# klausondrag/FOSVOS

Hardware: AMD Instinct MI355X
Metric: online fine-tune frames/sec (854x480) (higher is better)
Workload: dtype bf16; 1 GPU; OSVOS_VGG train_online one-shot fine-tune: 1x3x480x854 frame per step, fwd + class-balanced BCE + bwd, fused SGD step every 5 steps (BASELINE.json configs[1]); batch=1, avg_grad_every_n=5, activations=bf16 NHWC, fp32 accumulate, fp32 master weights, parallelism=single GPU

## Files before the change

### fosvos_amd/csrc/common.hpp

```cpp
#pragma once
#include <hip/hip_runtime.h>
#include <stdarg.h>
#include <algorithm>
#include <stdint.h>
#include <stdio.h>
#include <stdlib.h>
#include <string.h>

#include "../../include/fosvos_hip.h"

namespace fosvos {

extern thread_local char g_err[512];

inline int fail(int code, const char *fmt, ...) __attribute__((format(printf, 2, 3)));
inline int fail(int code, const char *fmt, ...) {
    va_list ap;
    va_start(ap, fmt);
    vsnprintf(g_err, sizeof(g_err), fmt, ap);
    va_end(ap);
    return code;
}

#define FOSVOS_HIP_CHECK(expr)                                                                         \
// ... 45 lines not shown
                     WgradReduceTable *reduce);
int wgrad_reduce_all(WgradReduceTable *reduce, int device, void *stream);
int wgrad_queue_reduce(const float *slabs, const float *bias_part, float *dw, float *db, int S, int S_bias, int64_t E_real,
                       int64_t E_pad, int Co, int Cor, int accumulate, WgradReduceTable *reduce, int device, void *stream);
struct HeadBwdArgs {
    const float *const *side;
    const int *hs, *ws;
    const float *const *filt, *const *filt1;
    const float *dsn_w, *fuse_w, *d_fused;
    const float *const *d_side_out;
    uint16_t *const *d_side;
    float *d_fuse_w, *d_fuse_b, *d_dsn_w, *d_dsn_b;
    int N, H, W, accumulate;
    void *workspace;
    size_t workspace_bytes;
    int device;
    int filt_uniform;
};
int head_bwd_check(const HeadBwdArgs &a);
int head_bwd_scale(const HeadBwdArgs &a, int s, void *stream);
int head_bwd_finish(const HeadBwdArgs &a, void *stream);

}
constexpr int kFosvosVggEvents = 25, kFosvosResnetEvents = 12;
struct fosvos_ctx {
    uint32_t magic;
    int device;
    hipEvent_t vgg_ev[kFosvosVggEvents];
    hipEvent_t resnet_ev[kFosvosResnetEvents];
    bool buckets_recorded;
};
constexpr uint32_t kFosvosCtxMagic = 0x58544346u;
namespace fosvos {
inline int ctx_check(const fosvos_ctx *ctx, const char *who) {
    FOSVOS_REQUIRE(ctx != nullptr, FOSVOS_E_ARG, "%s: null context (fosvos_ctx_create)", who);
    FOSVOS_REQUIRE(ctx->magic == kFosvosCtxMagic, FOSVOS_E_ARG, "%s: not a live fosvos_ctx", who);
    return FOSVOS_OK;
}

#ifdef FOSVOS_LAB_BUILD
inline const char *lab_env(const char *name) { return getenv(name); }
#else
inline const char *lab_env(const char *) { return nullptr; }
#endif
inline int lab_env_int(const char *name, int dflt) {
    const char *e = lab_env(name);
    return e ? atoi(e) : dflt;
}

bool conv_pp_applicable(int N, int H, int W, int in_ch, int out_ch);
int conv_pp_workgroups();
int conv_pp_forward(const uint16_t *x, const uint16_t *w_packed, const float *bias, uint16_t *y, uint16_t *y_pool, int N,
                    int H, int W, int Cin_pad, int Cout, int Co_pad, bool relu, hipStream_t st,
                    const uint8_t *mask_bits = nullptr);

inline int64_t cdiv(int64_t a, int64_t b) { return (a + b - 1) / b; }
inline int roundup(int a, int b) { return (a + b - 1) / b * b; }

typedef uint16_t bf16_t;
typedef __attribute__((ext_vector_type(8))) __bf16 bf16x8;
typedef __attribute__((ext_vector_type(4))) float f32x4;
typedef __attribute__((ext_vector_type(4))) short s16x4;
typedef unsigned int u32x4 __attribute__((__vector_size__(16)));

__device__ __forceinline__ uint16_t f2bf(float f) {
    __bf16 b = (__bf16)f;
    return __builtin_bit_cast(uint16_t, b);
}
__device__ __forceinline__ float bf2f(uint16_t v) { return __uint_as_float(((uint32_t)v) << 16); }
__device__ __forceinline__ uint4 repack8(const float (&f)[8]) {
    uint4 v;
    v.x = __builtin_amdgcn_perm(__float_as_uint(f[1]), __float_as_uint(f[0]), 0x07060302u);
    v.y = __builtin_amdgcn_perm(__float_as_uint(f[3]), __float_as_uint(f[2]), 0x07060302u);
    v.z = __builtin_amdgcn_perm(__float_as_uint(f[5]), __float_as_uint(f[4]), 0x07060302u);
    v.w = __builtin_amdgcn_perm(__float_as_uint(f[7]), __float_as_uint(f[6]), 0x07060302u);
    return v;
}
typedef float fosvos_f32x2 __attribute__((ext_vector_type(2)));
typedef __bf16 fosvos_bf16x2 __attribute__((ext_vector_type(2)));
__device__ __forceinline__ uint32_t pack2bf(float lo, float hi) {
    const fosvos_f32x2 v = {lo, hi};
    return __builtin_bit_cast(uint32_t, __builtin_convertvector(v, fosvos_bf16x2));
}
__device__ __forceinline__ float relu_f(float v) { return __int_as_float(max(__float_as_int(v), 0)); }
__device__ __forceinline__ void unpack8(const uint4 &v, float (&f)[8]) {
    f[0] = __uint_as_float(v.x << 16);
    f[1] = __uint_as_float(v.x & 0xffff0000u);
    f[2] = __uint_as_float(v.y << 16);
    f[3] = __uint_as_float(v.y & 0xffff0000u);
    f[4] = __uint_as_float(v.z << 16);
    f[5] = __uint_as_float(v.z & 0xffff0000u);
    f[6] = __uint_as_float(v.w << 16);
    f[7] = __uint_as_float(v.w & 0xffff0000u);
}
__device__ __forceinline__ uint4 pack8(const float (&f)[8]) {
    uint4 v;
    v.x = pack2bf(f[0], f[1]);
    v.y = pack2bf(f[2], f[3]);
    v.z = pack2bf(f[4], f[5]);
    v.w = pack2bf(f[6], f[7]);
    return v;
}

typedef short fosvos_i16x2 __attribute__((ext_vector_type(2)));
typedef unsigned short fosvos_u16x2 __attribute__((ext_vector_type(2)));
__device__ __forceinline__ uint32_t keep_where_pos_bf16x2(uint32_t f, uint32_t m) {
    const fosvos_i16x2 zero = {0, 0}, one = {1, 1};
// ... 91 lines not shown
```

### fosvos_amd/csrc/conv_igemm.hip

```cpp
#include <stdlib.h>

#include "common.hpp"

using namespace fosvos;

namespace {

constexpr unsigned kReluAfterAdd = 0x100u;
constexpr unsigned kSubsample2 = 0x200u;
constexpr unsigned kNoSplitK = 0x400u;

struct ConvArgs {
    const uint16_t *x;
    const uint16_t *w;
    const float *bias;
    const uint16_t *relu_src;
    const uint8_t *relu_bits;
    const uint16_t *addend;
    void *y;
    uint16_t *y_pool;
    const uint16_t *unpool_g;
    int N, H, W, Cin, Cout, Co_pad;
    int tiles_x, tiles_y;
    unsigned flags;
// ... 823 lines not shown
    if (int rc = check_common(x, w_packed, y, N, H, W, Ci, Co, "conv3x3_fwd_add")) return rc;
    FOSVOS_REQUIRE((flags & ~(FOSVOS_CONV_RELU | FOSVOS_CONV_OUT_F32)) == 0, FOSVOS_E_ARG, "conv3x3_fwd_add: unknown flags 0x%x",
                   flags);
    FOSVOS_REQUIRE(Co % 64 == 0 || Co == 32 || (Co == 16 && !addend), FOSVOS_E_SHAPE,
                   "conv3x3_fwd_add: Co=%d must be 32 or a multiple of 64 (16 without an addend)", Co);
    FOSVOS_REQUIRE(!(flags & FOSVOS_CONV_OUT_F32) || (Co == 16 && !addend), FOSVOS_E_ARG,
                   "conv3x3_fwd_add: fp32 output is the 16-channel side_prep form");
    FOSVOS_ENTER(device);
    ConvArgs a{};
    a.x = x; a.w = w_packed; a.bias = bias; a.relu_src = nullptr; a.addend = addend; a.y = y;
    a.N = N; a.H = H; a.W = W; a.Cin = roundup(Ci, 32); a.Cout = Co; a.Co_pad = roundup(Co, 16);
    a.flags = kNoSplitK | (addend ? ((flags & FOSVOS_CONV_RELU) ? kReluAfterAdd : 0u) : flags);
    return dispatch(a, Ci, workspace, workspace_bytes, (hipStream_t)stream);
}

extern "C" int fosvos_conv3x3_s2_fwd(const uint16_t *x, const uint16_t *w_packed, const float *bias, uint16_t *y, int N,
                                     int H, int W, int Ci, int Co, unsigned flags, void *workspace, size_t workspace_bytes,
                                     int device, void *stream) {
    if (int rc = check_common(x, w_packed, y, N, H, W, Ci, Co, "conv3x3_s2_fwd")) return rc;
    FOSVOS_REQUIRE((flags & ~FOSVOS_CONV_RELU) == 0, FOSVOS_E_ARG, "conv3x3_s2_fwd: unknown flags 0x%x", flags);
    FOSVOS_REQUIRE(Co % 64 == 0 || Co == 32, FOSVOS_E_SHAPE, "conv3x3_s2_fwd: Co=%d must be 32 or a multiple of 64", Co);
    FOSVOS_ENTER(device);
    ConvArgs a{};
    a.x = x; a.w = w_packed; a.bias = bias; a.relu_src = nullptr; a.addend = nullptr; a.y = y;
    a.N = N; a.H = H; a.W = W; a.Cin = roundup(Ci, 32); a.Cout = Co; a.Co_pad = roundup(Co, 16);
    a.flags = flags | kSubsample2 | kNoSplitK;
    return dispatch(a, Ci, workspace, workspace_bytes, (hipStream_t)stream);
}

extern "C" int fosvos_conv3x3_fwd_pool(const uint16_t *x, const uint16_t *w_packed, const float *bias, uint16_t *y,
                                       uint16_t *y_pool, int N, int H, int W, int Ci, int Co, unsigned flags,
                                       void *workspace, size_t workspace_bytes, int device, void *stream) {
    if (int rc = check_common(x, w_packed, y, N, H, W, Ci, Co, "conv3x3_fwd_pool")) return rc;
    FOSVOS_REQUIRE(y_pool, FOSVOS_E_ARG, "conv3x3_fwd_pool: null pooled output");
    FOSVOS_REQUIRE((flags & ~FOSVOS_CONV_RELU) == 0, FOSVOS_E_ARG, "conv3x3_fwd_pool: unknown flags 0x%x", flags);
    FOSVOS_REQUIRE(Co % 64 == 0, FOSVOS_E_SHAPE, "conv3x3_fwd_pool: Co=%d must be a multiple of 64", Co);
    if ((flags & FOSVOS_CONV_RELU) && forward_takes_pp(N, H, W, Ci, Co, flags)) {
        FOSVOS_ENTER(device);
        return conv_pp_forward(x, w_packed, bias, y, y_pool, N, H, W, roundup(Ci, 32), Co, roundup(Co, 16), true,
                               (hipStream_t)stream);
    }
    if (make_plan(N, H, W, Ci, Co).k_splits > 1) {
        if (int rc = fosvos_conv3x3_fwd(x, w_packed, bias, y, N, H, W, Ci, Co, flags, workspace, workspace_bytes, device, stream))
            return rc;
        return fosvos_maxpool2x2_ceil_fwd(y, y_pool, N, H, W, Co, device, stream);
    }
    FOSVOS_ENTER(device);
    ConvArgs a{};
    a.x = x; a.w = w_packed; a.bias = bias; a.relu_src = nullptr; a.addend = nullptr; a.y = y; a.y_pool = y_pool;
    a.N = N; a.H = H; a.W = W; a.Cin = roundup(Ci, 32); a.Cout = Co; a.Co_pad = roundup(Co, 16); a.flags = flags;
    return dispatch(a, Ci, workspace, workspace_bytes, (hipStream_t)stream);
}

extern "C" int fosvos_conv3x3_dgrad_bits(const uint16_t *dy, const uint16_t *w_dgrad_packed, const uint8_t *relu_bits,
                                         const uint16_t *addend, uint16_t *dx, int N, int H, int W, int Ci, int Co,
                                         void *workspace, size_t workspace_bytes, int device, void *stream) {
    if (int rc = check_common(dy, w_dgrad_packed, dx, N, H, W, Co, Ci, "conv3x3_dgrad_bits")) return rc;
    FOSVOS_REQUIRE(relu_bits && Ci % 8 == 0, FOSVOS_E_ARG, "conv3x3_dgrad_bits: null mask or Ci=%d not a multiple of 8", Ci);
    FOSVOS_ENTER(device);
    if (!addend && lab_env_int("FOSVOS_PP_DGRAD", 1) != 0 && lab_env_int("FOSVOS_PP", -1) != 0 &&
        conv_pp_applicable(N, H, W, roundup(Co, 32), Ci))
        return conv_pp_forward(dy, w_dgrad_packed, nullptr, dx, nullptr, N, H, W, roundup(Co, 32), Ci, roundup(Ci, 16), false,
                               (hipStream_t)stream, relu_bits);
    ConvArgs a{};
    a.x = dy; a.w = w_dgrad_packed; a.bias = nullptr; a.relu_src = nullptr; a.relu_bits = relu_bits; a.addend = addend; a.y = dx;
    a.N = N; a.H = H; a.W = W; a.Cin = roundup(Co, 32); a.Cout = Ci; a.Co_pad = roundup(Ci, 16); a.flags = 0;
    return dispatch(a, Co, workspace, workspace_bytes, (hipStream_t)stream);
}

extern "C" int fosvos_conv3x3_dgrad_unpool(const uint16_t *dy, const uint16_t *w_dgrad_packed, const uint16_t *x,
                                           const uint16_t *d_pooled, uint16_t *dx, int N, int H, int W, int Ci, int Co,
                                           void *workspace, size_t workspace_bytes, int device, void *stream) {
    if (int rc = check_common(dy, w_dgrad_packed, dx, N, H, W, Co, Ci, "conv3x3_dgrad_unpool")) return rc;
    FOSVOS_REQUIRE(x && d_pooled && x != dx, FOSVOS_E_ARG, "conv3x3_dgrad_unpool: null or aliased pooled-map operands");
    FOSVOS_ENTER(device);
    const ConvPlan plan = make_plan(N, H, W, Co, Ci);
    const bool fused = Ci % 64 == 0 && plan.k_splits == 1 && (plan.tile == kBig || plan.tile == kSquare || plan.tile == kMid) &&
                       lab_env_int("FOSVOS_UNPOOL_FUSED", 1) != 0;
    if (!fused) {
        if (int rc = fosvos_maxpool2x2_ceil_bwd(x, d_pooled, dx, N, H, W, Ci, 1, device, stream)) return rc;
        return fosvos_conv3x3_dgrad(dy, w_dgrad_packed, x, dx, dx, N, H, W, Ci, Co, workspace, workspace_bytes, device, stream);
    }
    ConvArgs a{};
    a.x = dy; a.w = w_dgrad_packed; a.relu_src = x; a.unpool_g = d_pooled; a.y = dx;
    a.N = N; a.H = H; a.W = W; a.Cin = roundup(Co, 32); a.Cout = Ci; a.Co_pad = roundup(Ci, 16); a.flags = 0;
    return dispatch(a, Co, workspace, workspace_bytes, (hipStream_t)stream);
}

extern "C" int fosvos_conv3x3_dgrad(const uint16_t *dy, const uint16_t *w_dgrad_packed, const uint16_t *relu_src,
                                    const uint16_t *addend, uint16_t *dx, int N, int H, int W, int Ci, int Co,
                                    void *workspace, size_t workspace_bytes, int device, void *stream) {
    if (int rc = check_common(dy, w_dgrad_packed, dx, N, H, W, Co, Ci, "conv3x3_dgrad")) return rc;
    FOSVOS_ENTER(device);
    ConvArgs a{};
    a.x = dy; a.w = w_dgrad_packed; a.bias = nullptr; a.relu_src = relu_src; a.addend = addend; a.y = dx;
    a.N = N; a.H = H; a.W = W; a.Cin = roundup(Co, 32); a.Cout = Ci; a.Co_pad = roundup(Ci, 16); a.flags = 0;
    return dispatch(a, Co, workspace, workspace_bytes, (hipStream_t)stream);
}
```

### fosvos_amd/csrc/conv_pp.hip

```cpp
#include <stdlib.h>

#include "common.hpp"

using namespace fosvos;

namespace fosvos {
namespace pp {

constexpr int TH = 8, TW = 32, BN = 64;
constexpr int HALO_W = TW + 2, HALO_H = TH + 2, NPIX = HALO_W * HALO_H;
constexpr int A_BYTES = NPIX * 64;
constexpr int A_PIECES = (NPIX * 4 + 63) / 64;
constexpr int W_BYTES = 36 * BN * 16;
constexpr int LDS_W = 0, LDS_A = 2 * W_BYTES, LDS_BIAS = LDS_A + 4 * A_BYTES, LDS_BYTES = LDS_BIAS + BN * 4;
constexpr int NT = 512;
static_assert(LDS_BYTES <= 160 * 1024, "one workgroup per CU");

struct Args {
    const uint16_t *x;
    const uint16_t *w;
    const float *bias;
    uint16_t *y;
    uint16_t *y_pool;
    const uint8_t *mask_bits;
    int N, H, W, Cin, Cout, Co_pad;
    int tiles_x, tiles_y, n_tiles;
    int n_cb;
    unsigned long long *stamps;
    int lab;
};
#ifdef FOSVOS_LAB_BUILD
#define PP_LAB(bit) (a.lab & (bit))
#define PP_STAMP(idx_)                                                                                            \
    if (a.stamps && blockIdx.x < 8 && wm == 0 && lane == 0 && (idx_) < 512)                                       \
        a.stamps[(blockIdx.x * 2 + g) * 512 + (idx_)] = __builtin_amdgcn_s_memtime();
#else
#define PP_LAB(bit) 0
#define PP_STAMP(idx_)
#endif

#pragma clang diagnostic push
#pragma clang diagnostic ignored "-Winline-asm"
__device__ __forceinline__ void dma16(const __amdgpu_buffer_rsrc_t rsrc, unsigned lds_dst, unsigned voff, unsigned soff) {
    asm volatile("s_mov_b32 m0, %0\n\ts_nop 4\n\tbuffer_load_dwordx4 %1, %2, %3 offen lds"
                 :: "s"(lds_dst), "v"(voff), "s"(rsrc), "s"(soff) : "memory", "m0");
}
__device__ __forceinline__ void wait_vm0() { asm volatile("s_waitcnt vmcnt(0)" ::: "memory"); }
__device__ __forceinline__ void wait_all() { asm volatile("s_waitcnt vmcnt(0) lgkmcnt(0)" ::: "memory"); }
__device__ __forceinline__ void pp_barrier() {
    asm volatile("" ::: "memory");
    __builtin_amdgcn_s_barrier();
    asm volatile("" ::: "memory");
}
#pragma clang diagnostic pop

typedef __attribute__((address_space(3))) void lds_void;
typedef __attribute__((address_space(3))) const uint4 *lds_u4_ptr;

struct TileIt {
    int idx, n, ty, tx;
    int d_n, d_ty, d_tx, stride;
    int tiles_x, tiles_y, end;
    __device__ __forceinline__ void init(int first, int stride_, int tiles_x_, int tiles_y_, int end_) {
        tiles_x = tiles_x_; tiles_y = tiles_y_; end = end_; stride = stride_;
        idx = first;
        const int per_img = tiles_x * tiles_y;
        n = first / per_img;
        const int r = first - n * per_img;
        ty = r / tiles_x;
        tx = r - ty * tiles_x;
        d_n = stride / per_img;
        const int rs = stride - d_n * per_img;
        d_ty = rs / tiles_x;
        d_tx = rs - d_ty * tiles_x;
    }
    __device__ __forceinline__ void next() {
        idx += stride;
        tx += d_tx;
        const int cx = tx >= tiles_x;
        tx -= cx ? tiles_x : 0;
        ty += d_ty + cx;
        const int cy = ty >= tiles_y;
        ty -= cy ? tiles_y : 0;
        n += d_n + cy;
    }
    __device__ __forceinline__ bool valid() const { return idx < end; }
    __device__ __forceinline__ int y0() const { return ty * TH; }
    __device__ __forceinline__ int x0() const { return tx * TW; }
};

template <bool RELU, bool POOL, bool MASK = false>
__global__ __launch_bounds__(NT) __attribute__((amdgpu_waves_per_eu(2, 2))) void k_conv3x3_pp(const Args a) {
    extern __shared__ __attribute__((aligned(16))) char smem_pp[];
    const unsigned lds0 = __builtin_amdgcn_readfirstlane((unsigned)(size_t)(lds_void *)smem_pp);
    const int tid = threadIdx.x, lane = tid & 63;
    const int wave = __builtin_amdgcn_readfirstlane(tid >> 6);
    const int g = wave >> 2, wm = wave & 3;
    const int cl = lane & 15, kq = lane >> 4;
    const int H = a.H, W = a.W, Cin = a.Cin, Cout = a.Cout;
    const int NC = Cin >> 5;

    const int b = blockIdx.x, n_wg8 = gridDim.x >> 3;
    const int xcd = b & 7, j8 = b >> 3;
    const int cb = j8 % a.n_cb, jj = j8 / a.n_cb, S = n_wg8 / a.n_cb;
    const int t_begin = (int)(((int64_t)xcd * a.n_tiles) >> 3), t_end = (int)(((int64_t)(xcd + 1) * a.n_tiles) >> 3);
    const int span = t_end - t_begin;
    const int n_it = span > 2 * jj ? (span - 2 * jj + 2 * S - 1) / (2 * S) : 0;
    if (n_it == 0) return;
    const int K = n_it * NC;
    const int n0 = cb * BN;
    TileIt cur, ldt;
    cur.init(t_begin + 2 * jj + g, 2 * S, a.tiles_x, a.tiles_y, t_end);
    ldt = cur;

    const int pj = lane >> 4, pm = lane & 15;
    const unsigned w_voff = (unsigned)(32 * (pj >> 1) + 8 * (pm >> 2) + 4 * (pj & 1) + (pm & 3)) * 16u;
    const int w_row_bytes = a.Co_pad * 16;
    const auto w_rsrc = __builtin_amdgcn_make_buffer_rsrc(const_cast<uint16_t *>(a.w), 0, NC * 36 * w_row_bytes, 0x00020000);
    auto issue_w = [&](int chunk, int buf, int first, int stride) {
        if (PP_LAB(8)) return;
        for (int r = first; r < 36; r += stride)
            dma16(w_rsrc, lds0 + LDS_W + buf * W_BYTES + r * 1024, w_voff, (unsigned)((chunk * 36 + r) * w_row_bytes + n0 * 16));
    };

    constexpr int A_IT = (A_PIECES + 3) / 4;
    int a_rel[A_IT];
#pragma unroll
    for (int i = 0; i < A_IT; ++i) {
        const int pc = wm + 4 * i;
        const int P = pc * 16 + (lane >> 2), s4 = lane & 3;
        const int hy = P / HALO_W, hx = P - hy * HALO_W;
        const int kq_src = s4 ^ ((P >> 1) & 2);
        a_rel[i] = (hy * W + hx) * Cin * 2 + kq_src * 16;
    }
    int ld_k = 0, ld_c = 0;
    int ld_base = 0, ld_edge = 0;
    __amdgpu_buffer_rsrc_t ld_rsrc;
    auto ld_open_tile = [&]() {
        if (!ldt.valid()) return;
        const int y0 = ldt.y0(), x0 = ldt.x0();
        ld_rsrc = __builtin_amdgcn_make_buffer_rsrc(const_cast<uint16_t *>(a.x) + (int64_t)ldt.n * H * W * Cin, 0,
                                                    H * W * Cin * 2, 0x00020000);
        ld_base = ((y0 - 1) * W + (x0 - 1)) * Cin * 2;
        ld_edge = !(y0 > 0 && x0 > 0 && y0 + TH < H && x0 + TW < W);
// ... 53 lines not shown
    af[i_] = __builtin_bit_cast(bf16x8, *(lds_u4_ptr)(size_t)(lds0 + LDS_A + (g * 2 + ((k_) & 1)) * A_BYTES +  \
                                                              a_sw[((i_) >> 1) + (tap_) / 3][(tap_) % 3] + ((i_) & 1) * 1024));
#define PP_RW(k_, tap_, s_, j_) \
    wf[s_][j_] = __builtin_bit_cast(bf16x8, *(lds_u4_ptr)(size_t)(w_frag0 + ((k_) & 1) * W_BYTES + (tap_) * 4096 + (j_) * 256));
#define PP_RBIAS()                                                                                            \
    _Pragma("unroll") for (int i = 0; i < 4; ++i) _Pragma("unroll") for (int j = 0; j < 4; ++j) acc[i][j] =    \
        *(__attribute__((address_space(3))) const f32x4 *)(size_t)(bias_at + (j >> 1) * 128 + (j & 1) * 16);

    uint4 pk[4][2];
    unsigned mb[MASK ? 4 : 1][2];
    int dn_n = 0, dn_y0 = 0, dn_x0 = 0;
    int st_pending = 0;
    auto pack_frag = [&](int i, int jp) {
        unsigned u[4];
#pragma unroll
        for (int e2 = 0; e2 < 4; ++e2) {
            const int e = 2 * e2;
            u[e2] = pack2bf(acc[i][2 * jp + (e >> 2)][e & 3], acc[i][2 * jp + (e >> 2)][(e & 3) + 1]);
            if constexpr (RELU) {
                const fosvos_i16x2 zero = {0, 0};
                u[e2] = __builtin_bit_cast(unsigned, __builtin_elementwise_max(__builtin_bit_cast(fosvos_i16x2, u[e2]), zero));
            }
        }
        return make_uint4(u[0], u[1], u[2], u[3]);
    };
    auto pack_tile = [&]() {
        if (!cur.valid() || PP_LAB(2)) return;
        dn_n = cur.n; dn_y0 = cur.y0(); dn_x0 = cur.x0();
        st_pending = 1;
#pragma unroll
        for (int i = 0; i < 4; ++i) {
            pk[i][0] = pack_frag(i, 0);
            pk[i][1] = pack_frag(i, 1);
        }
        if constexpr (MASK) {
            const auto m_rsrc = __builtin_amdgcn_make_buffer_rsrc(const_cast<uint8_t *>(a.mask_bits) + (int64_t)dn_n * H * W * (Cout >> 3),
                                                                  0, H * W * (Cout >> 3), 0x00020000);
#pragma unroll
            for (int i = 0; i < 4; ++i) {
                const int gy = dn_y0 + 2 * wm + (i >> 1), gx = dn_x0 + (i & 1) * 16 + cl;
                const unsigned off = (gy < H && gx < W) ? (unsigned)((gy * W + gx) * (Cout >> 3) + (n0 >> 3) + kq) : 0x80000000u;
                mb[i][0] = __builtin_amdgcn_raw_buffer_load_b8(m_rsrc, off, 0, 0);
                mb[i][1] = __builtin_amdgcn_raw_buffer_load_b8(m_rsrc, off + 4, 0, 0);
            }
        }
    };
    auto mask_bits_of = [](unsigned b) {
        return make_uint4((b & 1u) | ((b & 2u) << 15), ((b >> 2) & 1u) | ((b & 8u) << 13), ((b >> 4) & 1u) | ((b & 32u) << 11),
                          ((b >> 6) & 1u) | ((b & 128u) << 9));
    };
    auto store_slot = [&](int slot) {
        if (!st_pending) return;
        if (slot < 4) {
            const auto y_rsrc = __builtin_amdgcn_make_buffer_rsrc(a.y + (int64_t)dn_n * H * W * Cout, 0, H * W * Cout * 2, 0x00020000);
            const int gy = dn_y0 + 2 * wm + (slot >> 1), gx = dn_x0 + (slot & 1) * 16 + cl;
            const unsigned off = (gy < H && gx < W) ? (unsigned)(((gy * W + gx) * Cout + n0 + kq * 8) * 2) : 0x80000000u;
            uint4 v0 = pk[slot][0], v1 = pk[slot][1];
            if constexpr (MASK) {
                v0 = keep_where_pos_bf16x8(v0, mask_bits_of(mb[slot][0]));
                v1 = keep_where_pos_bf16x8(v1, mask_bits_of(mb[slot][1]));
            }
            __builtin_amdgcn_raw_buffer_store_b128(__builtin_bit_cast(u32x4, v0), y_rsrc, off, 0, 0);
            __builtin_amdgcn_raw_buffer_store_b128(__builtin_bit_cast(u32x4, v1), y_rsrc, off + 64, 0, 0);
        } else if constexpr (POOL) {
            const int ih = slot - 4;
            const int OH = (H + 1) >> 1, OW = (W + 1) >> 1;
            const bool edge = dn_y0 + TH > H || dn_x0 + TW > W;
            const auto p_rsrc = __builtin_amdgcn_make_buffer_rsrc(a.y_pool + (int64_t)dn_n * OH * OW * Cout, 0,
                                                                  OH * OW * Cout * 2, 0x00020000);
            const int oy = (dn_y0 >> 1) + wm, ox = (dn_x0 >> 1) + ih * 8 + (cl >> 1);
            const bool ok = !(cl & 1) && oy < OH && ox < OW;
            const unsigned off = ok ? (unsigned)(((oy * OW + ox) * Cout + n0 + kq * 8) * 2) : 0x80000000u;
#pragma unroll
            for (int jp = 0; jp < 2; ++jp) {
                uint4 top = pk[ih][jp], bot = pk[ih + 2][jp];
                if (edge) {
                    const int gy = dn_y0 + 2 * wm, gx = dn_x0 + ih * 16 + cl;
                    if (!(gy < H && gx < W)) top = make_uint4(0, 0, 0, 0);
                    if (!(gy + 1 < H && gx < W)) bot = make_uint4(0, 0, 0, 0);
                }
                const uint4 m = max_nonneg_bf16x8(top, bot);
                uint4 o;
                o.x = (unsigned)__builtin_amdgcn_update_dpp(0, (int)m.x, 0xB1, 0xF, 0xF, true);
                o.y = (unsigned)__builtin_amdgcn_update_dpp(0, (int)m.y, 0xB1, 0xF, 0xF, true);
                o.z = (unsigned)__builtin_amdgcn_update_dpp(0, (int)m.z, 0xB1, 0xF, 0xF, true);
                o.w = (unsigned)__builtin_amdgcn_update_dpp(0, (int)m.w, 0xB1, 0xF, 0xF, true);
                __builtin_amdgcn_raw_buffer_store_b128(__builtin_bit_cast(u32x4, max_nonneg_bf16x8(m, o)), p_rsrc, off + jp * 64, 0, 0);
            }
        }
    };
    constexpr int N_SLOTS = POOL ? 6 : 4;

    auto request_next = [&](int k) {
        if (k + 1 < K && (NC > 2 || k + 1 < 2)) issue_w((k + 1) % NC, (k + 1) & 1, wave, 8);
        ld_issue();
    };

    issue_w(0, 0, wave, 8);
    ld_open_tile();
    ld_issue();
    wait_all();
    pp_barrier();

#define PP_MM(tap_, i_, j_) \
    acc[i_][j_] = __builtin_amdgcn_mfma_f32_16x16x32_bf16(wf[(tap_) & 1][j_], af[i_], acc[i_][j_], 0, 0, 0);
#define PP_ROW_READS(n_, i_)                                                                                  \
    PP_RA(k, n_, i_)                                                                                          \
    if constexpr ((i_) < 2) {                                                                                 \
        PP_RW(k, n_, (n_) & 1, 2 * (i_))                                                                      \
        PP_RW(k, n_, (n_) & 1, 2 * (i_) + 1)                                                                  \
    }                                                                                                         \
    __builtin_amdgcn_sched_group_barrier(0x008, 4, 0);                                                        \
    __builtin_amdgcn_sched_group_barrier(0x002, 1, 0);                                                        \
    __builtin_amdgcn_sched_group_barrier(0x100, (i_) < 2 ? 3 : 1, 0);
#define PP_ROW(tap_, i_)                                                                                      \
    PP_MM(tap_, i_, 0) PP_MM(tap_, i_, 1) PP_MM(tap_, i_, 2) PP_MM(tap_, i_, 3)                               \
    PP_ROW_READS((tap_) + 1, i_)
#define PP_TAP(tap_) { PP_ROW(tap_, 0) PP_ROW(tap_, 1) PP_ROW(tap_, 2) PP_ROW(tap_, 3) }
#define PP_TAP_LAST()                                                                                         \
    {                                                                                                         \
// ... 26 lines not shown
            PP_BETWEEN(0) PP_BETWEEN(1) PP_BETWEEN(2) PP_BETWEEN(3) PP_BETWEEN(4) PP_BETWEEN(5) PP_BETWEEN(6) PP_BETWEEN(7) PP_BETWEEN(8)
        }
        st_pending = 0;
        if (++cp_c == NC) {
            cp_c = 0;
            pack_tile();
            cur.next();
        }
        PP_STAMP(4 * k + 2)
        wait_vm0();
        PP_STAMP(4 * k + 3)
        pp_barrier();
    }
    PP_STAMP(4 * K)
#pragma unroll
    for (int slot = 0; slot < N_SLOTS; ++slot) store_slot(slot);
#undef PP_MM
#undef PP_ROW_READS
#undef PP_ROW
#undef PP_TAP
#undef PP_TAP_LAST
#undef PP_BETWEEN
#undef PP_RA
#undef PP_RW
#undef PP_RBIAS
}

}
}

namespace fosvos {
int conv_pp_workgroups() { return 256; }
#ifdef FOSVOS_LAB_BUILD
static unsigned long long *g_pp_stamps = nullptr;
extern "C" void fosvos_lab_set_pp_stamps(void *p) { g_pp_stamps = (unsigned long long *)p; }
#endif

bool conv_pp_applicable(int N, int H, int W, int in_ch, int out_ch) {
    if (out_ch % 64 != 0 || in_ch % 32 != 0) return false;
    const int n_cb = out_ch / 64;
    if (n_cb != 1 && n_cb != 2 && n_cb != 4 && n_cb != 8) return false;
    const int64_t tiles = cdiv(W, pp::TW) * cdiv(H, pp::TH) * N;
    if (tiles > 0x3fffffff) return false;
    const int64_t units = tiles * n_cb, slots = 2 * conv_pp_workgroups();
    if (units < slots) return false;
    static const int mode = lab_env_int("FOSVOS_PP", -1);
    if (mode == 1 || in_ch <= 64) return true;
    return units * 10 >= cdiv(units, slots) * slots * 9;
}



int conv_pp_forward(const uint16_t *x, const uint16_t *w_packed, const float *bias, uint16_t *y, uint16_t *y_pool, int N,
                    int H, int W, int Cin_pad, int Cout, int Co_pad, bool relu, hipStream_t st, const uint8_t *mask_bits) {
    FOSVOS_REQUIRE(!y_pool || relu, FOSVOS_E_ARG, "conv3x3 (persistent): the fused pool takes post-ReLU values");
    FOSVOS_REQUIRE(!mask_bits || (!relu && !y_pool && !bias), FOSVOS_E_ARG, "conv3x3 (persistent): the bit mask is the data gradient's epilogue");
    pp::Args a{};
    a.x = x; a.w = w_packed; a.bias = bias; a.y = y; a.y_pool = y_pool; a.mask_bits = mask_bits;
    a.N = N; a.H = H; a.W = W; a.Cin = Cin_pad; a.Cout = Cout; a.Co_pad = Co_pad;
    a.tiles_x = (int)cdiv(W, pp::TW);
    a.tiles_y = (int)cdiv(H, pp::TH);
    a.n_tiles = a.tiles_x * a.tiles_y * N;
    a.n_cb = Cout / 64;
    a.lab = lab_env_int("FOSVOS_PP_LAB", 0);
#ifdef FOSVOS_LAB_BUILD
    a.stamps = g_pp_stamps;
#endif
    void (*kern)(const pp::Args) = mask_bits ? pp::k_conv3x3_pp<false, false, true>
                                   : y_pool  ? pp::k_conv3x3_pp<true, true>
                                   : relu    ? pp::k_conv3x3_pp<true, false> : pp::k_conv3x3_pp<false, false>;
    const int which = mask_bits ? 3 : y_pool ? 2 : relu ? 1 : 0;
    static bool once[64][4];
    int dev = 0;
    FOSVOS_HIP_CHECK(hipGetDevice(&dev));
    if (dev >= 0 && dev < 64 && !once[dev][which]) {
        FOSVOS_HIP_CHECK(hipFuncSetAttribute(reinterpret_cast<const void *>(kern), hipFuncAttributeMaxDynamicSharedMemorySize,
                                             pp::LDS_BYTES));
        once[dev][which] = true;
    }
    FOSVOS_PROF(mask_bits ? "k_conv3x3_pp<false, false, true>" : y_pool ? "k_conv3x3_pp<true, true, false>"
                : relu    ? "k_conv3x3_pp<true, false, false>" : "k_conv3x3_pp<false, false, false>", st,
                2.0 * N * H * W * 9.0 * Cin_pad * Cout);
    hipLaunchKernelGGL(kern, dim3(conv_pp_workgroups()), dim3(pp::NT), pp::LDS_BYTES, st, a);
    FOSVOS_LAUNCH_CHECK();
    return FOSVOS_OK;
}

}
```

### fosvos_amd/csrc/pool.hip

```cpp
#include "common.hpp"

using namespace fosvos;

namespace {
__global__ __launch_bounds__(256) void k_pool_fwd(const uint16_t *__restrict__ x, uint16_t *__restrict__ y, int H,
                                                   int W, int C, int OH, int OW, int64_t total) {
    const int groups = C >> 3;
    for (int64_t i = blockIdx.x * (int64_t)blockDim.x + threadIdx.x; i < total; i += (int64_t)gridDim.x * blockDim.x) {
        const int g = (int)(i % groups);
        int64_t r = i / groups;
        const int ox = (int)(r % OW);
        r /= OW;
        const int oy = (int)(r % OH);
        const int64_t n = r / OH;
        const int iy = oy * 2, ix = ox * 2;
        float m[8];
#pragma unroll
        for (int j = 0; j < 8; ++j) m[j] = -INFINITY;
#pragma unroll
        for (int dy = 0; dy < 2; ++dy)
#pragma unroll
            for (int dx = 0; dx < 2; ++dx) {
                if (iy + dy < H && ix + dx < W) {
                    const uint4 v = *reinterpret_cast<const uint4 *>(
// ... 6 lines not shown
            }
        *reinterpret_cast<uint4 *>(y + (((n * OH + oy) * OW + ox) * C + g * 8)) = pack8(m);
    }
}

__global__ __launch_bounds__(256) void k_pool_bwd(const uint16_t *__restrict__ x, const uint16_t *__restrict__ dy,
                                                   uint16_t *__restrict__ dx, int H, int W, int C, int OH, int OW,
                                                   int relu_mask) {
    const int groups = C >> 3;
    const int col = blockIdx.x * 256 + threadIdx.x;
    if (col >= OW * groups) return;
    const int ox = col / groups, g = col - ox * groups;
    const int oy = blockIdx.y;
    const int64_t n = blockIdx.z;
    const uint16_t *xn = x + n * H * W * C;
    uint16_t *dxn = dx + n * H * W * C;
    const int iy = oy * 2, ix = ox * 2;
    const bool vx = ix + 1 < W, vy = iy + 1 < H;
    const int o00 = (iy * W + ix) * C + g * 8;
    const int o01 = o00 + C, o10 = o00 + W * C, o11 = o10 + C;
    const uint4 v0 = *reinterpret_cast<const uint4 *>(xn + o00);
    const uint4 v1 = *reinterpret_cast<const uint4 *>(xn + (vx ? o01 : o00));
    const uint4 v2 = *reinterpret_cast<const uint4 *>(xn + (vy ? o10 : o00));
    const uint4 v3 = *reinterpret_cast<const uint4 *>(xn + (vx && vy ? o11 : o00));
    const uint4 gv = *reinterpret_cast<const uint4 *>(dy + ((n * OH + oy) * OW + ox) * C + g * 8);
    float x0[8], x1[8], x2[8], x3[8], gy[8];
    unpack8(v0, x0);
    unpack8(v1, x1);
    unpack8(v2, x2);
    unpack8(v3, x3);
    unpack8(gv, gy);
    float r0[8], r1[8], r2[8], r3[8];
#pragma unroll
    for (int j = 0; j < 8; ++j) {
        const float a1 = vx ? x1[j] : -INFINITY, a2 = vy ? x2[j] : -INFINITY, a3 = (vx && vy) ? x3[j] : -INFINITY;
        const bool w1 = a1 > x0[j];
        const float m1 = w1 ? a1 : x0[j];
        const bool w2 = a2 > m1;
        const float m2 = w2 ? a2 : m1;
        const bool w3 = a3 > m2;
        const float m = w3 ? a3 : m2;
        const float gval = (relu_mask && !(m > 0.f)) ? 0.f : gy[j];
        r0[j] = (w1 || w2 || w3) ? 0.f : gval;
        r1[j] = (w1 && !w2 && !w3) ? gval : 0.f;
        r2[j] = (w2 && !w3) ? gval : 0.f;
        r3[j] = w3 ? gval : 0.f;
    }
    *reinterpret_cast<uint4 *>(dxn + o00) = repack8(r0);
    if (vx) *reinterpret_cast<uint4 *>(dxn + o01) = repack8(r1);
    if (vy) *reinterpret_cast<uint4 *>(dxn + o10) = repack8(r2);
    if (vx && vy) *reinterpret_cast<uint4 *>(dxn + o11) = repack8(r3);
}

inline int grid_for(int64_t total) {
    int64_t g = cdiv(total, 256);
    if (g > 16384) g = 16384;
    if (g < 1) g = 1;
    return (int)g;
}
}

extern "C" int fosvos_maxpool2x2_ceil_fwd(const uint16_t *x, uint16_t *y, int N, int H, int W, int C, int device,
                                          void *stream) {
    FOSVOS_REQUIRE(x && y, FOSVOS_E_ARG, "maxpool_fwd: null pointer");
    FOSVOS_REQUIRE(N > 0 && H > 0 && W > 0 && C > 0 && C % 8 == 0, FOSVOS_E_SHAPE,
                   "maxpool_fwd: bad shape N=%d H=%d W=%d C=%d (C %% 8 must be 0)", N, H, W, C);
    FOSVOS_ENTER(device);
    const int OH = (H + 1) / 2, OW = (W + 1) / 2;
    const int64_t total = (int64_t)N * OH * OW * (C / 8);
    FOSVOS_PROF("k_pool_fwd", stream, 0.0);
    hipLaunchKernelGGL(k_pool_fwd, dim3(grid_for(total)), dim3(256), 0, (hipStream_t)stream, x, y, H, W, C, OH, OW, total);
    FOSVOS_LAUNCH_CHECK();
    return FOSVOS_OK;
}

extern "C" int fosvos_maxpool2x2_ceil_bwd(const uint16_t *x, const uint16_t *dy, uint16_t *dx, int N, int H, int W,
                                          int C, int relu_mask, int device, void *stream) {
    FOSVOS_REQUIRE(x && dy && dx, FOSVOS_E_ARG, "maxpool_bwd: null pointer");
    FOSVOS_REQUIRE(N > 0 && H > 0 && W > 0 && C > 0 && C % 8 == 0, FOSVOS_E_SHAPE,
                   "maxpool_bwd: bad shape N=%d H=%d W=%d C=%d (C %% 8 must be 0)", N, H, W, C);
    FOSVOS_ENTER(device);
    const int OH = (H + 1) / 2, OW = (W + 1) / 2;
    FOSVOS_REQUIRE((int64_t)H * W * C < 0x7fffffffLL && OH <= 65535 && N <= 65535, FOSVOS_E_SHAPE,
                   "maxpool_bwd: image too large (N=%d H=%d W=%d C=%d)", N, H, W, C);
    FOSVOS_PROF("k_pool_bwd", stream, 0.0);
    hipLaunchKernelGGL(k_pool_bwd, dim3((unsigned)cdiv((int64_t)OW * (C / 8), 256), (unsigned)OH, (unsigned)N), dim3(256), 0,
                       (hipStream_t)stream, x, dy, dx, H, W, C, OH, OW, relu_mask);
    FOSVOS_LAUNCH_CHECK();
    return FOSVOS_OK;
}
```

### fosvos_amd/csrc/vgg_net.hip

```cpp
#include <stdlib.h>

#include "common.hpp"

using namespace fosvos;

namespace {
constexpr int kNConv = 13;
constexpr int kStageOf[kNConv] = {0, 0, 1, 1, 2, 2, 2, 3, 3, 3, 4, 4, 4};
constexpr int kCin[kNConv] = {3, 64, 64, 128, 128, 256, 256, 256, 512, 512, 512, 512, 512};
constexpr int kCout[kNConv] = {64, 64, 128, 128, 256, 256, 256, 512, 512, 512, 512, 512, 512};
constexpr int kFirstOfStage[5] = {0, 2, 4, 7, 10};
constexpr int kLastOfStage[5] = {1, 3, 6, 9, 12};
constexpr int kStageCh[5] = {64, 128, 256, 512, 512};

inline size_t up256(size_t v) { return (v + 255) / 256 * 256; }

struct Arena {
    int sh[5], sw[5];
    size_t act[kNConv];
    size_t gact[kNConv];
    size_t pooled[4];
    size_t gpooled[4];
    size_t side[4];
    size_t dside[4];
// ... 18 lines not shown
    }
    for (int s = 1; s < 5; ++s) {
        const size_t bytes = (size_t)N * a.sh[s] * a.sw[s] * kStageCh[s - 1] * 2;
        a.pooled[s - 1] = take(bytes);
        a.gpooled[s - 1] = take(bytes);
        a.side[s - 1] = take((size_t)N * a.sh[s] * a.sw[s] * 16 * 4);
        a.dside[s - 1] = take((size_t)N * a.sh[s] * a.sw[s] * 32 * 2);
    }
    a.bits0 = take((size_t)N * H * W * (kCout[0] / 8));
    a.hws_bytes = up256(fosvos_head_bwd_workspace_bytes(N, H, W));
    a.hws = take(a.hws_bytes);
    size_t ws = 256;
    a.wsa_conv_bytes[0] = up256(fosvos_conv3x3_first_wgrad_workspace_bytes(N, H, W, 64));
    for (int c = 1; c < kNConv; ++c) {
        const int s = kStageOf[c];
        a.wsa_conv_bytes[c] = fosvos_conv3x3_wgrad_workspace_bytes(N, a.sh[s], a.sw[s], kCin[c], kCout[c]);
        if (N >= 2)
            a.wsa_conv_bytes[c] = std::max(a.wsa_conv_bytes[c],
                                           fosvos_conv3x3_workspace_bytes(N - (N + 1) / 2, a.sh[s], a.sw[s], kCin[c], kCout[c]));
        a.wsa_conv_bytes[c] = up256(a.wsa_conv_bytes[c]);
        ws = std::max(ws, fosvos_conv3x3_workspace_bytes(N, a.sh[s], a.sw[s], kCin[c], kCout[c]));
        if (N >= 2)
            ws = std::max(ws, fosvos_conv3x3_workspace_bytes((N + 1) / 2, a.sh[s], a.sw[s], kCin[c], kCout[c]));
        ws = std::max(ws, fosvos_conv3x3_workspace_bytes(N, a.sh[s], a.sw[s], kCout[c], kCin[c]));
    }
    for (int s = 1; s < 5; ++s) {
        a.wsa_side_bytes[s - 1] = up256(std::max({fosvos_conv3x3_wgrad_workspace_bytes(N, a.sh[s], a.sw[s], kStageCh[s], 16),
                                                  fosvos_conv3x3_workspace_bytes(N, a.sh[s], a.sw[s], kStageCh[s], 16),
                                                  N >= 2 ? fosvos_conv3x3_workspace_bytes(N - (N + 1) / 2, a.sh[s], a.sw[s], kStageCh[s], 16) : (size_t)0}));
        ws = std::max(ws, fosvos_conv3x3_workspace_bytes(N, a.sh[s], a.sw[s], kStageCh[s], 16));
        if (N >= 2) ws = std::max(ws, fosvos_conv3x3_workspace_bytes((N + 1) / 2, a.sh[s], a.sw[s], kStageCh[s], 16));
        ws = std::max(ws, fosvos_conv3x3_workspace_bytes(N, a.sh[s], a.sw[s], 16, kStageCh[s]));
    }
    a.ws_bytes = up256(ws);
    a.ws = take(a.ws_bytes);
    for (int c = 0; c < kNConv; ++c) a.wsa_conv[c] = take(a.wsa_conv_bytes[c]);
    for (int i = 0; i < 4; ++i) a.wsa_side[i] = take(a.wsa_side_bytes[i]);
    a.total = off;
    return a;
}

static_assert(kFosvosVggEvents == 25, "event slots below");
constexpr int kBucketFinalEvent = 22;
constexpr int kStage2WgradEvent = 23;
constexpr int kMainTailEvent = 24;
constexpr int kBucketEvent0 = 19;

#define FOSVOS_TRY(expr)          \
    do {                          \
        const int rc_ = (expr);   \
        if (rc_ != FOSVOS_OK) return rc_; \
    } while (0)

int check_net(const void *w, const void *frame, const void *arena, int N, int H, int W, size_t arena_bytes,
              const Arena &a, const char *who) {
    FOSVOS_REQUIRE(w && frame && arena, FOSVOS_E_ARG, "%s: null pointer", who);
    FOSVOS_REQUIRE(N > 0 && H > 0 && W > 0, FOSVOS_E_SHAPE, "%s: bad shape N=%d H=%d W=%d", who, N, H, W);
    FOSVOS_REQUIRE(arena_bytes >= a.total, FOSVOS_E_WORKSPACE, "%s: arena %zu < %zu bytes", who, arena_bytes, a.total);
    FOSVOS_REQUIRE(((uintptr_t)arena & 255) == 0, FOSVOS_E_ARG, "%s: arena must be 256-byte aligned", who);
    return FOSVOS_OK;
}
}

extern "C" size_t fosvos_vgg_arena_bytes(int N, int H, int W) {
    if (N <= 0 || H <= 0 || W <= 0) return 0;
    return make_arena(N, H, W).total;
}

extern "C" int fosvos_vgg_arena_layout(int N, int H, int W, fosvos_vgg_arena_layout_info *out) {
    FOSVOS_REQUIRE(out, FOSVOS_E_ARG, "vgg_arena_layout: null output");
    FOSVOS_REQUIRE(N > 0 && H > 0 && W > 0, FOSVOS_E_SHAPE, "vgg_arena_layout: bad shape N=%d H=%d W=%d", N, H, W);
    const Arena a = make_arena(N, H, W);
    *out = fosvos_vgg_arena_layout_info{};
    out->total = a.total;
    for (int s = 0; s < 5; ++s) { out->stage_h[s] = a.sh[s]; out->stage_w[s] = a.sw[s]; }
    for (int c = 0; c < kNConv; ++c) {
        const int s = kStageOf[c];
        out->act[c] = a.act[c];
        out->gact[c] = a.gact[c];
        out->act_bytes[c] = (size_t)N * a.sh[s] * a.sw[s] * kCout[c] * 2;
        out->wsa_conv[c] = a.wsa_conv[c];
        out->wsa_conv_bytes[c] = a.wsa_conv_bytes[c];
    }
    for (int s = 1; s < 5; ++s) {
        const size_t px = (size_t)N * a.sh[s] * a.sw[s];
        out->pooled[s - 1] = a.pooled[s - 1];
        out->gpooled[s - 1] = a.gpooled[s - 1];
        out->pooled_bytes[s - 1] = px * kStageCh[s - 1] * 2;
        out->side[s - 1] = a.side[s - 1];
        out->side_bytes[s - 1] = px * 16 * 4;
        out->dside[s - 1] = a.dside[s - 1];
        out->dside_bytes[s - 1] = px * 32 * 2;
        out->wsa_side[s - 1] = a.wsa_side[s - 1];
        out->wsa_side_bytes[s - 1] = a.wsa_side_bytes[s - 1];
    }
    out->bits0 = a.bits0;
    out->bits0_bytes = (size_t)N * H * W * (kCout[0] / 8);
    out->ws = a.ws; out->ws_bytes = a.ws_bytes;
    out->hws = a.hws; out->hws_bytes = a.hws_bytes;
    return FOSVOS_OK;
}

namespace {
int forward_impl(hipEvent_t *ev, const fosvos_vgg_weights *w, const float *frame, int N, int H, int W, void *arena,
                 size_t arena_bytes, float *fused, float *const side_out[4], int device, void *stream, void *aux_stream) {
    const Arena a = make_arena(N, H, W);
    FOSVOS_TRY(check_net(w, frame, arena, N, H, W, arena_bytes, a, "vgg_forward"));
    FOSVOS_REQUIRE(fused, FOSVOS_E_ARG, "vgg_forward: null output");
    char *base = reinterpret_cast<char *>(arena);
    auto act = [&](int c) { return reinterpret_cast<uint16_t *>(base + a.act[c]); };
    void *ws = base + a.ws;
    hipStream_t sm = (hipStream_t)stream;
    const bool par = ev != nullptr && aux_stream != nullptr && aux_stream != stream;
    hipStream_t sa = par ? (hipStream_t)aux_stream : sm;
    if (par) FOSVOS_ENTER(device);
    static const bool split_on = lab_env_int("FOSVOS_FWD_SPLIT", 1) != 0;
    if (split_on && N >= 2) {
        const int na = (N + 1) / 2;
        if (par) {
            FOSVOS_HIP_CHECK(hipEventRecord(ev[14], sm));
            FOSVOS_HIP_CHECK(hipStreamWaitEvent(sa, ev[14], 0));
        }
        for (int half = 0; half < 2; ++half) {
            const int f0 = half ? na : 0, nf = half ? N - na : na;
            hipStream_t st = half ? sa : sm;
            const uint16_t *xh = nullptr;
            for (int c = 0; c < kNConv; ++c) {
                const int s = kStageOf[c];
                const size_t px = (size_t)a.sh[s] * a.sw[s];
                uint16_t *yc = act(c) + (size_t)f0 * px * kCout[c];
                void *wsc = half ? base + a.wsa_conv[c] : ws;
                const size_t wsn = half ? a.wsa_conv_bytes[c] : a.ws_bytes;
                if (c == 0) {
                    FOSVOS_TRY(fosvos_conv3x3_first_fwd(frame + (size_t)f0 * 3 * H * W, w->conv_w[0], w->conv_b[0], yc,
                                                        reinterpret_cast<uint8_t *>(base + a.bits0) + (size_t)f0 * px * (kCout[0] / 8),
                                                        nf, H, W, kCout[0], device, st));
                } else {
                    if (c == kFirstOfStage[s]) {
                        const size_t ppx = (size_t)a.sh[s] * a.sw[s];
                        xh = reinterpret_cast<uint16_t *>(base + a.pooled[s - 1]) + (size_t)f0 * ppx * kCin[c];
                    }
                    FOSVOS_REQUIRE(wsn >= fosvos_conv3x3_workspace_bytes(nf, a.sh[s], a.sw[s], kCin[c], kCout[c]),
                                   FOSVOS_E_WORKSPACE, "vgg_forward: split-K workspace of the second chain");
                    if (c == kLastOfStage[s] && s < 4) {
                        const size_t qpx = (size_t)a.sh[s + 1] * a.sw[s + 1];
                        FOSVOS_TRY(fosvos_conv3x3_fwd_pool(xh, w->conv_wf[c], w->conv_b[c], yc,
                                                           reinterpret_cast<uint16_t *>(base + a.pooled[s]) + (size_t)f0 * qpx * kCout[c],
                                                           nf, a.sh[s], a.sw[s], kCin[c], kCout[c], FOSVOS_CONV_RELU, wsc, wsn,
                                                           device, st));
                    } else {
                        FOSVOS_TRY(fosvos_conv3x3_fwd(xh, w->conv_wf[c], w->conv_b[c], yc, nf, a.sh[s], a.sw[s], kCin[c],
                                                      kCout[c], FOSVOS_CONV_RELU, wsc, wsn, device, st));
                    }
                }
                xh = yc;
                if (s > 0 && c == kLastOfStage[s]) {
                    float *so = reinterpret_cast<float *>(base + a.side[s - 1]) + (size_t)f0 * px * 16;
                    FOSVOS_TRY(fosvos_conv3x3_fwd(xh, w->side_wf[s - 1], w->side_b[s - 1], so, nf, a.sh[s], a.sw[s], kStageCh[s],
                                                  16, FOSVOS_CONV_OUT_F32, half ? base + a.wsa_side[s - 1] : ws,
                                                  half ? a.wsa_side_bytes[s - 1] : a.ws_bytes, device, st));
                }
            }
        }
        static const bool head_per_chain = lab_env_int("FOSVOS_HEAD_PER_CHAIN", 1) != 0;
        if (head_per_chain) {
            for (int half = 0; half < 2; ++half) {
                const int f0 = half ? na : 0, nf = half ? N - na : na;
                const float *sideh[4];
                float *soh[4] = {nullptr, nullptr, nullptr, nullptr};
                int hsh[4], wsh[4];
                for (int i = 0; i < 4; ++i) {
                    hsh[i] = a.sh[i + 1];
                    wsh[i] = a.sw[i + 1];
                    sideh[i] = reinterpret_cast<const float *>(base + a.side[i]) + (size_t)f0 * hsh[i] * wsh[i] * 16;
                    if (side_out && side_out[i]) soh[i] = side_out[i] + (size_t)f0 * H * W;
                }
                FOSVOS_TRY(fosvos_head_fwd(sideh, hsh, wsh, w->filt, w->filt1, w->dsn_w, w->dsn_b, w->fuse_w, w->fuse_b,
                                           fused + (size_t)f0 * H * W, (side_out && side_out[0]) ? soh : nullptr, nf, H, W,
                                           w->filt_uniform, device, half ? sa : sm));
            }
        }
        if (par) {
            FOSVOS_HIP_CHECK(hipEventRecord(ev[13], sa));
            FOSVOS_HIP_CHECK(hipStreamWaitEvent(sm, ev[13], 0));
        }
        if (head_per_chain) return FOSVOS_OK;
    } else {
    const uint16_t *x = nullptr;
    for (int c = 0; c < kNConv; ++c) {
        const int s = kStageOf[c];
        if (c == 0) {
            FOSVOS_TRY(fosvos_conv3x3_first_fwd(frame, w->conv_w[0], w->conv_b[0], act(0),
                                                reinterpret_cast<uint8_t *>(base + a.bits0), N, H, W, kCout[0], device, stream));
        } else {
            if (c == kFirstOfStage[s])
                x = reinterpret_cast<uint16_t *>(base + a.pooled[s - 1]);
            if (c == kLastOfStage[s] && s < 4) {
                FOSVOS_TRY(fosvos_conv3x3_fwd_pool(x, w->conv_wf[c], w->conv_b[c], act(c),
                                                   reinterpret_cast<uint16_t *>(base + a.pooled[s]), N, a.sh[s], a.sw[s],
                                                   kCin[c], kCout[c], FOSVOS_CONV_RELU, ws, a.ws_bytes, device, stream));
            } else {
                FOSVOS_TRY(fosvos_conv3x3_fwd(x, w->conv_wf[c], w->conv_b[c], act(c), N, a.sh[s], a.sw[s], kCin[c], kCout[c],
                                              FOSVOS_CONV_RELU, ws, a.ws_bytes, device, stream));
            }
        }
        x = act(c);
        if (s > 0 && c == kLastOfStage[s]) {
            const bool on_aux = par && s < 4;
            if (on_aux) {
                FOSVOS_HIP_CHECK(hipEventRecord(ev[c], sm));
                FOSVOS_HIP_CHECK(hipStreamWaitEvent(sa, ev[c], 0));
            }
            FOSVOS_TRY(fosvos_conv3x3_fwd(x, w->side_wf[s - 1], w->side_b[s - 1], base + a.side[s - 1], N, a.sh[s], a.sw[s],
                                          kStageCh[s], 16, FOSVOS_CONV_OUT_F32, on_aux ? base + a.wsa_side[s - 1] : ws,
                                          on_aux ? a.wsa_side_bytes[s - 1] : a.ws_bytes, device, on_aux ? sa : sm));
        }
    }
    if (par) {
        FOSVOS_HIP_CHECK(hipEventRecord(ev[13], sa));
        FOSVOS_HIP_CHECK(hipStreamWaitEvent(sm, ev[13], 0));
    }
    }
    const float *side[4];
    int hs[4], wsz[4];
    for (int i = 0; i < 4; ++i) {
        side[i] = reinterpret_cast<const float *>(base + a.side[i]);
        hs[i] = a.sh[i + 1];
        wsz[i] = a.sw[i + 1];
    }
    return fosvos_head_fwd(side, hs, wsz, w->filt, w->filt1, w->dsn_w, w->dsn_b, w->fuse_w, w->fuse_b, fused, side_out, N, H,
                           W, w->filt_uniform, device, stream);
}
}

extern "C" int fosvos_vgg_forward_streams(fosvos_ctx *ctx, const fosvos_vgg_weights *w, const float *frame, int N, int H,
                                          int W, void *arena, size_t arena_bytes, float *fused, float *const side_out[4],
                                          void *stream, void *aux_stream) {
    FOSVOS_TRY(ctx_check(ctx, "vgg_forward_streams"));
    return forward_impl(ctx->vgg_ev, w, frame, N, H, W, arena, arena_bytes, fused, side_out, ctx->device, stream, aux_stream);
}

extern "C" int fosvos_vgg_forward(const fosvos_vgg_weights *w, const float *frame, int N, int H, int W, void *arena,
                                  size_t arena_bytes, float *fused, float *const side_out[4], int device,
                                  void *stream) {
    return forward_impl(nullptr, w, frame, N, H, W, arena, arena_bytes, fused, side_out, device, stream, nullptr);
}

extern "C" int fosvos_vgg_backward(fosvos_ctx *ctx, const fosvos_vgg_weights *w, const fosvos_vgg_grads *g,
                                   const float *frame, int N, int H, int W, void *arena, size_t arena_bytes,
                                   const float *d_fused, const float *const d_side_out[4], void *stream,
                                   void *aux_stream) {
    FOSVOS_TRY(ctx_check(ctx, "vgg_backward"));
    const int device = ctx->device;
    const Arena a = make_arena(N, H, W);
    FOSVOS_TRY(check_net(w, frame, arena, N, H, W, arena_bytes, a, "vgg_backward"));
    FOSVOS_REQUIRE(g, FOSVOS_E_ARG, "vgg_backward: null gradient table");
    const bool with_so = d_side_out && d_side_out[0];
    FOSVOS_REQUIRE(d_fused || with_so, FOSVOS_E_ARG, "vgg_backward: no upstream gradient given");
    char *base = reinterpret_cast<char *>(arena);
    auto act = [&](int c) { return reinterpret_cast<uint16_t *>(base + a.act[c]); };
    auto gact = [&](int c) { return reinterpret_cast<uint16_t *>(base + a.gact[c]); };
    void *ws = base + a.ws;
    const int acc = g->accumulate ? 1 : 0;
    WgradReduceTable reduce;
    reduce.n = 0;
    WgradReduceTable reduce_m;
    reduce_m.n = 0;

    hipStream_t sm = (hipStream_t)stream;
    const bool par = aux_stream != nullptr && aux_stream != stream;
    hipStream_t sa = par ? (hipStream_t)aux_stream : sm;
    hipEvent_t *ev = ctx->vgg_ev;
    const bool buckets = g->bucket_events != 0;
    const bool tail = g->last_pass_of_cycle != 0;
    static const int tail_stages = lab_env_int("FOSVOS_TAIL_STAGES", 1);
    static const bool offload_on = lab_env_int("FOSVOS_TAIL_OFFLOAD", 1) != 0;
    const bool offload = tail && aux_stream != nullptr && aux_stream != stream && offload_on;
    FOSVOS_ENTER(device);
    ctx->buckets_recorded = false;
    if (par) {
        FOSVOS_HIP_CHECK(hipEventRecord(ev[14], sm));
        FOSVOS_HIP_CHECK(hipStreamWaitEvent(sa, ev[14], 0));
    }
    auto publish = [&](int e) -> int {
        if (!par) return FOSVOS_OK;
        FOSVOS_HIP_CHECK(hipEventRecord(ev[e], sm));
        FOSVOS_HIP_CHECK(hipStreamWaitEvent(sa, ev[e], 0));
        return FOSVOS_OK;
    };

    const float *side[4];
    uint16_t *dside[4];
    int hs[4], wsz[4];
    for (int i = 0; i < 4; ++i) {
        side[i] = reinterpret_cast<const float *>(base + a.side[i]);
        dside[i] = reinterpret_cast<uint16_t *>(base + a.dside[i]);
        hs[i] = a.sh[i + 1];
        wsz[i] = a.sw[i + 1];
    }
    const HeadBwdArgs ha{side, hs, wsz, w->filt, with_so ? w->filt1 : nullptr, with_so ? w->dsn_w : nullptr, w->fuse_w,
                         d_fused, with_so ? d_side_out : nullptr, dside, g->fuse_w, g->fuse_b,
                         with_so ? g->dsn_w : nullptr, with_so ? g->dsn_b : nullptr, N, H, W, acc, base + a.hws,
                         a.hws_bytes, device, w->filt_uniform & 15};
    FOSVOS_TRY(head_bwd_check(ha));
    FOSVOS_TRY(head_bwd_scale(ha, 3, sm));
// ... 5 lines not shown
    FOSVOS_TRY(head_bwd_finish(ha, sa));

    static const bool unpool_fused = lab_env_int("FOSVOS_UNPOOL", 1) != 0;
    for (int s = 4; s >= 0; --s) {
        const int hh = a.sh[s], ww = a.sw[s], last = kLastOfStage[s], first = kFirstOfStage[s];
        if (s > 0) {
            FOSVOS_TRY(wgrad_impl(act(last), dside[s - 1], g->side_w[s - 1], g->side_b[s - 1], N, hh, ww, kStageCh[s], 16,
                                  acc, base + a.wsa_side[s - 1], a.wsa_side_bytes[s - 1], device, sa,
                                  (offload && s == 1) ? &reduce_m : &reduce, tail && s <= tail_stages));
            const uint16_t *addend = (s < 4) ? gact(last) : nullptr;
            if (par && s < 4) FOSVOS_HIP_CHECK(hipStreamWaitEvent(sm, ev[16 + s - 1], 0));
            if (s < 4 && unpool_fused)
                FOSVOS_TRY(fosvos_conv3x3_dgrad_unpool(dside[s - 1], w->side_wd[s - 1], act(last),
                                                       reinterpret_cast<const uint16_t *>(base + a.gpooled[s]), gact(last), N, hh,
                                                       ww, kStageCh[s], 16, ws, a.ws_bytes, device, sm));
            else
                FOSVOS_TRY(fosvos_conv3x3_dgrad(dside[s - 1], w->side_wd[s - 1], act(last), addend, gact(last), N, hh, ww,
                                                kStageCh[s], 16, ws, a.ws_bytes, device, sm));
        }
        FOSVOS_TRY(publish(last));
        for (int c = last; c >= first; --c) {
            if (c == 0) {
                if (offload)
                    FOSVOS_TRY(first_wgrad_impl(frame, gact(0), g->conv_w[0], g->conv_b[0], N, H, W, kCout[0], acc,
                                                base + a.wsa_conv[0], a.wsa_conv_bytes[0], device, sm, &reduce_m));
                else
                    FOSVOS_TRY(first_wgrad_impl(frame, gact(0), g->conv_w[0], g->conv_b[0], N, H, W, kCout[0], acc,
                                                base + a.wsa_conv[0], a.wsa_conv_bytes[0], device, sa, &reduce));
                break;
            }
            const bool from_pool = (c == first) && s > 0;
            const uint16_t *xin = from_pool ? reinterpret_cast<const uint16_t *>(base + a.pooled[s - 1]) : act(c - 1);
            uint16_t *dx = from_pool ? reinterpret_cast<uint16_t *>(base + a.gpooled[s - 1]) : gact(c - 1);
            const uint16_t *mask = from_pool ? nullptr : act(c - 1);
            const bool middle = (last - first == 2) && c == last - 1;
            if (!middle)
                FOSVOS_TRY(wgrad_impl(xin, gact(c), g->conv_w[c], g->conv_b[c], N, hh, ww, kCin[c], kCout[c], acc,
                                      base + a.wsa_conv[c], a.wsa_conv_bytes[c], device, sa,
                                      (offload && s == 1) ? &reduce_m : &reduce, tail && s <= tail_stages));
            static const bool bits_on = lab_env_int("FOSVOS_RELU_BITS", 1) != 0;
            if (c == 1 && bits_on)
                FOSVOS_TRY(fosvos_conv3x3_dgrad_bits(gact(c), w->conv_wd[c], reinterpret_cast<const uint8_t *>(base + a.bits0), nullptr,
                                                     dx, N, hh, ww, kCin[c], kCout[c], ws, a.ws_bytes, device, sm));
            else
                FOSVOS_TRY(fosvos_conv3x3_dgrad(gact(c), w->conv_wd[c], mask, nullptr, dx, N, hh, ww, kCin[c], kCout[c], ws,
                                                a.ws_bytes, device, sm));
            const bool skip_event = (last - first == 2) && c == last;
            if (!from_pool && !skip_event) FOSVOS_TRY(publish(c - 1));
            if (middle)
                FOSVOS_TRY(wgrad_impl(xin, gact(c), g->conv_w[c], g->conv_b[c], N, hh, ww, kCin[c], kCout[c], acc,
                                      base + a.wsa_conv[c], a.wsa_conv_bytes[c], device, sa,
                                      (offload && s == 1) ? &reduce_m : &reduce, tail && s <= tail_stages));
        }
        if (s == 1 || (s > 0 && !unpool_fused))
            FOSVOS_TRY(fosvos_maxpool2x2_ceil_bwd(act(kLastOfStage[s - 1]), reinterpret_cast<const uint16_t *>(base + a.gpooled[s - 1]),
                                                  gact(kLastOfStage[s - 1]), N, a.sh[s - 1], a.sw[s - 1], kStageCh[s - 1], 1,
                                                  device, sm));
        if (s >= 1) {
            FOSVOS_TRY(wgrad_reduce_all(&reduce, device, sa));
            if (buckets && s >= 2) FOSVOS_HIP_CHECK(hipEventRecord(ev[kBucketEvent0 + (4 - s)], sa));
            if (offload && s == 1) FOSVOS_HIP_CHECK(hipEventRecord(ev[kStage2WgradEvent], sa));
        }
    }
    FOSVOS_TRY(wgrad_reduce_all(&reduce, device, sa));
    if (offload) {
        FOSVOS_HIP_CHECK(hipStreamWaitEvent(sm, ev[kStage2WgradEvent], 0));
        FOSVOS_TRY(wgrad_reduce_all(&reduce_m, device, sm));
    }
    if (buckets) FOSVOS_HIP_CHECK(hipEventRecord(ev[kMainTailEvent], sm));
    if (buckets) {
        FOSVOS_HIP_CHECK(hipEventRecord(ev[kBucketFinalEvent], sa));
        ctx->buckets_recorded = true;
    }
    if (par && !g->defer_join) {
        FOSVOS_HIP_CHECK(hipEventRecord(ev[15], sa));
        FOSVOS_HIP_CHECK(hipStreamWaitEvent(sm, ev[15], 0));
    }
    return FOSVOS_OK;
}

extern "C" int fosvos_vgg_grad_bucket_wait(fosvos_ctx *ctx, int bucket, void *stream) {
    FOSVOS_TRY(ctx_check(ctx, "vgg_grad_bucket_wait"));
    FOSVOS_REQUIRE(bucket >= 0 && bucket < 5, FOSVOS_E_ARG, "vgg_grad_bucket_wait: bucket %d not in 0..4", bucket);
    FOSVOS_ENTER(ctx->device);
    FOSVOS_REQUIRE(ctx->buckets_recorded, FOSVOS_E_ARG,
                   "vgg_grad_bucket_wait: the last fosvos_vgg_backward on this context did not set grads.bucket_events");
    hipEvent_t *ev = ctx->vgg_ev;
    if (bucket < 3) {
        FOSVOS_HIP_CHECK(hipStreamWaitEvent((hipStream_t)stream, ev[kBucketEvent0 + bucket], 0));
    } else {
        FOSVOS_HIP_CHECK(hipStreamWaitEvent((hipStream_t)stream, ev[kBucketFinalEvent], 0));
        FOSVOS_HIP_CHECK(hipStreamWaitEvent((hipStream_t)stream, ev[kMainTailEvent], 0));
    }
    return FOSVOS_OK;
}
```

### fosvos_amd/fosvos_hip/__init__.py

```python
from __future__ import annotations

import ctypes
import os
import threading
from ctypes import POINTER, c_char_p, c_float, c_int, c_int64, c_size_t, c_uint, c_void_p

_HERE = os.path.dirname(os.path.abspath(__file__))
PKG_ROOT = os.path.dirname(_HERE)
LIB_PATH = os.environ.get("FOSVOS_HIP_LIB") or os.path.join(PKG_ROOT, "lib", "libfosvos_hip.so")
HEADER_PATH = os.path.join(os.path.dirname(PKG_ROOT), "include", "fosvos_hip.h")

ABI_VERSION = 33
CONV_RELU = 1
CONV_OUT_F32 = 2


class FosvosHipError(RuntimeError):
    pass


class SgdEntry(ctypes.Structure):
    _fields_ = [("param", c_void_p), ("grad", c_void_p), ("momentum_buf", c_void_p), ("numel", c_int64),
                ("lr", c_float), ("weight_decay", c_float)]


_P4 = c_void_p * 4
_I4 = c_int * 4
_P13 = c_void_p * 13


class VggWeights(ctypes.Structure):
    _fields_ = [("conv_w", _P13), ("conv_b", _P13), ("conv_wf", _P13), ("conv_wd", _P13),
                ("side_b", _P4), ("side_wf", _P4), ("side_wd", _P4), ("filt", _P4), ("filt1", _P4),
                ("dsn_w", c_void_p), ("dsn_b", c_void_p), ("fuse_w", c_void_p), ("fuse_b", c_void_p),
                ("filt_uniform", c_int)]


class VggGrads(ctypes.Structure):
    _fields_ = [("conv_w", _P13), ("conv_b", _P13), ("side_w", _P4), ("side_b", _P4),
                ("dsn_w", c_void_p), ("dsn_b", c_void_p), ("fuse_w", c_void_p), ("fuse_b", c_void_p),
                ("accumulate", c_int), ("defer_join", c_int), ("bucket_events", c_int), ("last_pass_of_cycle", c_int)]

_Z4 = c_size_t * 4
_Z13 = c_size_t * 13


class VggArenaLayout(ctypes.Structure):
    _fields_ = [("total", c_size_t), ("stage_h", c_int * 5), ("stage_w", c_int * 5),
                ("act", _Z13), ("gact", _Z13), ("act_bytes", _Z13),
                ("pooled", _Z4), ("gpooled", _Z4), ("pooled_bytes", _Z4),
                ("side", _Z4), ("side_bytes", _Z4), ("dside", _Z4), ("dside_bytes", _Z4),
                ("bits0", c_size_t), ("bits0_bytes", c_size_t),
                ("ws", c_size_t), ("ws_bytes", c_size_t), ("hws", c_size_t), ("hws_bytes", c_size_t),
                ("wsa_conv", _Z13), ("wsa_conv_bytes", _Z13), ("wsa_side", _Z4), ("wsa_side_bytes", _Z4)]


class Conv3x3PlanInfo(ctypes.Structure):
    _fields_ = [("tile_h", c_int), ("tile_w", c_int), ("tile_co", c_int), ("k_splits", c_int), ("workgroups", c_int),
                ("persistent", c_int)]


class Conv2dPlanInfo(ctypes.Structure):
    _fields_ = [("cob", c_int), ("threads", c_int), ("slices", c_int), ("workgroups", c_int), ("mfma_frag_blocks", c_int),
                ("mfma_workgroups", c_int)]


class ProfileRecord(ctypes.Structure):
# ... 122 lines not shown
    "fosvos_vgg_forward_streams": (c_int, [c_void_p, POINTER(VggWeights), c_void_p, c_int, c_int, c_int, c_void_p, c_size_t,
                                           c_void_p, POINTER(c_void_p), c_void_p, c_void_p]),
    "fosvos_augment_sample": (c_int, [c_void_p, c_void_p, c_int, c_int, c_int, c_void_p, c_void_p, c_void_p, c_void_p,
                                      c_void_p, c_void_p, c_int, c_int, c_void_p, c_void_p, c_void_p, c_void_p, c_int,
                                      c_void_p]),
    "fosvos_prob_bytes": (c_int, [c_void_p, c_int, c_int, c_int, c_void_p, c_void_p, c_int, c_void_p]),
    "fosvos_jf_workspace_bytes": (c_size_t, [c_int, c_int, c_int]),
    "fosvos_jf_counts": (c_int, [c_void_p, c_void_p, c_int, c_int, c_int, c_int, c_void_p, c_void_p, c_size_t, c_int,
                                 c_void_p]),
    "fosvos_png_capacity_bytes": (c_size_t, [c_int, c_int, c_int]),
    "fosvos_png_workspace_bytes": (c_size_t, [c_int, c_int, c_int, c_int]),
    "fosvos_png_encode": (c_int, [c_void_p, c_int, c_int, c_int, c_int, c_void_p, c_size_t, c_void_p, c_void_p, c_size_t, c_int,
                                  c_void_p]),
    "fosvos_merge_objects": (c_int, [POINTER(c_void_p), c_int, c_int, c_int, c_int, c_void_p, c_int, c_void_p]),
    "fosvos_jf_labels_workspace_bytes": (c_size_t, [c_int, c_int, c_int, c_int]),
    "fosvos_jf_counts_labels": (c_int, [c_void_p, c_void_p, c_int, c_int, c_int, c_int, c_int, c_void_p, c_void_p, c_size_t,
                                        c_int, c_void_p]),
    "fosvos_components_workspace_bytes": (c_size_t, [c_int, c_int, c_int]),
    "fosvos_component_roots": (c_int, [c_void_p, c_int, c_int, c_int, c_void_p, c_void_p, c_size_t, c_int, c_void_p]),
    "fosvos_clean_components": (c_int, [c_void_p, c_void_p, c_int, c_int, c_int, c_int, c_int, c_int, c_int, c_float, c_void_p,
                                        c_void_p, c_void_p, c_size_t, c_int, c_void_p]),
    "fosvos_cbce_void_workspace_bytes": (c_size_t, [c_int64, c_int]),
    "fosvos_cbce_loss_frames_void": (c_int, [c_void_p, c_void_p, c_void_p, c_int64, c_int, c_int, c_float, c_void_p, c_void_p,
                                             c_void_p, c_size_t, c_int, c_void_p]),
    "fosvos_distance_gate_workspace_bytes": (c_size_t, [c_int, c_int, c_int]),
    "fosvos_distance_gate": (c_int, [c_void_p, c_int, c_int, c_int, c_int, c_int, c_void_p, c_void_p, c_size_t, c_int,
                                     c_void_p]),
    "fosvos_adapt_labels_workspace_bytes": (c_size_t, [c_int, c_int, c_int]),
    "fosvos_adapt_labels": (c_int, [c_void_p, c_void_p, c_int, c_int, c_int, c_float, c_int, c_int, c_void_p, c_void_p,
                                    c_void_p, c_void_p, c_size_t, c_int, c_void_p]),
    "fosvos_png_indexed_capacity_bytes": (c_size_t, [c_int, c_int, c_int]),
    "fosvos_png_encode_indexed": (c_int, [c_void_p, c_void_p, c_int, c_int, c_int, c_int, c_void_p, c_size_t, c_void_p,
                                          c_void_p, c_size_t, c_int, c_void_p]),
    "fosvos_jpeg_capacity_bytes": (c_size_t, [c_int, c_int, c_int, c_int, c_int]),
    "fosvos_jpeg_workspace_bytes": (c_size_t, [c_int, c_int, c_int, c_int, c_int]),
    "fosvos_jpeg_encode": (c_int, [c_void_p, c_int, c_int, c_int, c_int, c_int, c_int, c_void_p, c_size_t, c_void_p, c_void_p,
                                   c_size_t, c_int, c_void_p]),
    "fosvos_jpeg_decode_workspace_bytes": (c_size_t, [c_int, c_int, c_int, c_int, c_int]),
    "fosvos_jpeg_decode": (c_int, [c_void_p, c_size_t, c_void_p, c_int, c_void_p, c_int, c_int, c_int, c_int, c_int, c_void_p,
                                   c_void_p, c_void_p, c_size_t, c_int, c_void_p]),
    "fosvos_frame_prep": (c_int, [c_void_p, c_int, c_int, c_int, c_int, POINTER(c_float), c_void_p, c_int, c_void_p]),
    "fosvos_overlay": (c_int, [c_void_p, c_void_p, c_int, c_int, c_int, c_int, c_int, c_int, ctypes.c_double, c_void_p, c_int,
                               c_void_p]),
    "fosvos_frame_prep_scaled": (c_int, [c_void_p, c_int, c_int, c_int, c_int, c_int, c_int, POINTER(c_float), c_void_p, c_int,
                                         c_void_p]),
    "fosvos_overlay_scaled": (c_int, [c_void_p, c_void_p, c_int, c_int, c_int, c_int, c_int, c_int, c_int, c_int,
                                      ctypes.c_double, c_void_p, c_int, c_void_p]),
    "fosvos_overlay_objects": (c_int, [c_void_p, POINTER(c_void_p), c_int, c_int, c_int, c_int, c_int, c_void_p,
                                       ctypes.c_double, c_void_p, c_int, c_void_p]),
    "fosvos_overlay_objects_scaled": (c_int, [c_void_p, POINTER(c_void_p), c_int, c_int, c_int, c_int, c_int, c_int, c_int,
                                              c_int, c_void_p, ctypes.c_double, c_void_p, c_int, c_void_p]),
    "fosvos_vgg_backward": (c_int, [c_void_p, POINTER(VggWeights), POINTER(VggGrads), c_void_p, c_int, c_int, c_int, c_void_p,
                                    c_size_t, c_void_p, POINTER(c_void_p), c_void_p, c_void_p]),
}

_lib = None
_lock = threading.Lock()


def lib() -> ctypes.CDLL:
    global _lib
    if _lib is not None:
        return _lib
    with _lock:
        if _lib is not None:
            return _lib
        if not os.path.exists(LIB_PATH):
            raise FosvosHipError(
                f"{LIB_PATH} not found: build it with `python -c 'import __graft_entry__ as g; g.build()'` "
                f"or `make -C fosvos_amd/csrc`.  There is no CPU fallback.")
        import torch
        handle = ctypes.CDLL(LIB_PATH)
        for name, (restype, argtypes) in SIGNATURES.items():
            fn = getattr(handle, name)
            fn.restype = restype
            fn.argtypes = argtypes
        got = handle.fosvos_abi_version()
        if got != ABI_VERSION:
            raise FosvosHipError(f"libfosvos_hip.so ABI {got} != binding ABI {ABI_VERSION}: rebuild")
        _lib = handle
    return _lib


def check(rc: int, what: str) -> None:
    if rc != 0:
        msg = lib().fosvos_last_error()
        raise FosvosHipError(f"{what} failed (code {rc}): {msg.decode(errors='replace') if msg else ''}")


class LaunchProfile:

    def __init__(self, device: int, max_launches: int = 65536):
        self.device, self.max_launches, self.records = int(device), int(max_launches), {}

    def __enter__(self):
        check(lib().fosvos_profile_start(self.device, self.max_launches), "profile_start")
        return self

    def __exit__(self, *exc):
        buf = (ProfileRecord * 128)()
        n = c_int(0)
        check(lib().fosvos_profile_stop(self.device, buf, 128, ctypes.byref(n)), "profile_stop")
        self.records = {buf[i].name.decode(): {"launches": buf[i].launches, "ms": buf[i].ms, "flops": buf[i].flops}
                        for i in range(n.value)}
        return False

# ... 27 lines not shown
```

### fosvos_amd/fosvos_hip/engine.py

```python
from __future__ import annotations

import ctypes
import time
from dataclasses import dataclass
from typing import Dict, List, Optional, Sequence, Tuple

import torch

from . import Context, VggGrads, VggWeights, check, lib, ops, ptr_array4
from .options import EngineOptions, native_loop_from_env

STAGE_CHANNELS = ((64, 64), (128, 128), (256, 256, 256), (512, 512, 512), (512, 512, 512))
STAGE_IN = (3, 64, 128, 256, 512)
SIDE_CH = 16


def conv_module_index(stage: int, k: int) -> int:
    return 2 * k + (0 if stage == 0 else 1)


def param_names() -> List[str]:
    names = [f"upscale.{i}.weight" for i in range(4)] + [f"upscale_.{i}.weight" for i in range(4)]
    for s, chans in enumerate(STAGE_CHANNELS):
        for j in range(len(chans)):
            m = conv_module_index(s, j)
            names += [f"stages.{s}.{m}.weight", f"stages.{s}.{m}.bias"]
    for i in range(4):
        names += [f"side_prep.{i}.weight", f"side_prep.{i}.bias"]
    for i in range(4):
        names += [f"score_dsn.{i}.weight", f"score_dsn.{i}.bias"]
    names += ["fuse.weight", "fuse.bias"]
    return names


PARAM_NAMES = param_names()
PARAM_INDEX = {n: i for i, n in enumerate(PARAM_NAMES)}


@dataclass(slots=True)
class PassFlags:

    defer_wgrad_join: bool = False
    forward_one_stream: bool = False
    publish_grad_buckets: bool = False
    overwrite_grads: bool = False
    last_pass_of_cycle: bool = False


class PackedWeights:

    def __init__(self, options: Optional[EngineOptions] = None) -> None:
        self.options = options if options is not None else EngineOptions.from_env()
        self.flags = PassFlags()
        self._cache: Dict[str, Tuple[object, object, object]] = {}
        self._uniform: Dict[str, bool] = {}
        self.arenas = ArenaPool()

    @staticmethod
    def _key(t: torch.Tensor) -> Tuple[int, int]:
        return (t.data_ptr(), t._version)

    def invalidate(self) -> None:
        self._cache.clear()
        self._uniform.clear()

    def small(self, name: str, parts: Sequence[torch.Tensor]) -> torch.Tensor:
        key = tuple(self._key(t) for t in parts)
        hit = self._cache.get(name)
        if hit is not None and hit[0] == key:
            return hit[1]
        cat = torch.cat([t.detach().reshape(-1) for t in parts]).contiguous()
        self._cache[name] = (key, cat, tuple(t.untyped_storage() for t in parts))
        return cat

    def conv(self, name: str, w: torch.Tensor):
        key = self._key(w)
        hit = self._cache.get(name)
        if hit is not None and hit[0] == key:
            return hit[1]
        packed = ops.pack_conv3x3_weights(w.detach(), True, True)
        self._cache[name] = (key, packed, w.untyped_storage())
        return packed

    def conv_many(self, named: Sequence[Tuple[str, torch.Tensor]]):
        stale = []
        for name, w in named:
            hit = self._cache.get(name)
            if hit is None or hit[0] != self._key(w):
                stale.append((name, w))
        if stale:
            packed = ops.pack_conv3x3_weights_multi([w.detach() for _, w in stale])
            for (name, w), pk in zip(stale, packed):
                self._cache[name] = (self._key(w), pk, w.untyped_storage())
        return [self._cache[name][1] for name, _ in named]

    def deconv_diag(self, name: str, w: torch.Tensor) -> torch.Tensor:
        key = self._key(w)
        hit = self._cache.get(name)
        if hit is not None and hit[0] == key:
# ... 306 lines not shown
def _aligned_ptr(arena: torch.Tensor) -> Tuple[int, int]:
    p = arena.data_ptr()
    ap = (p + 255) // 256 * 256
    return ap, arena.numel() - (ap - p)


def _weights_struct(P: Dict[str, torch.Tensor], packs: PackedWeights):
    w = VggWeights()
    keep = []
    named = [(wn, P[wn]) for c, (wn, _) in enumerate(_CONV_NAMES) if c > 0]
    named += [(f"side_prep.{i}.weight", P[f"side_prep.{i}.weight"]) for i in range(4)]
    images = packs.conv_many(named)
    for c, (wn, bn) in enumerate(_CONV_NAMES):
        w.conv_w[c] = P[wn].data_ptr()
        w.conv_b[c] = P[bn].data_ptr()
        if c > 0:
            wf, wd = images[c - 1]
            w.conv_wf[c], w.conv_wd[c] = wf.data_ptr(), wd.data_ptr()
    for i in range(4):
        wf, wd = images[len(_CONV_NAMES) - 1 + i]
        w.side_wf[i], w.side_wd[i] = wf.data_ptr(), wd.data_ptr()
        w.side_b[i] = P[f"side_prep.{i}.bias"].data_ptr()
        f = packs.deconv_diag(f"upscale.{i}.weight", P[f"upscale.{i}.weight"])
        f1 = packs.deconv_diag(f"upscale_.{i}.weight", P[f"upscale_.{i}.weight"])
        w.filt[i], w.filt1[i] = f.data_ptr(), f1.data_ptr()
    dsn_w = packs.small("dsn_w", [P[f"score_dsn.{i}.weight"] for i in range(4)])
    dsn_b = packs.small("dsn_b", [P[f"score_dsn.{i}.bias"] for i in range(4)])
    w.dsn_w, w.dsn_b = dsn_w.data_ptr(), dsn_b.data_ptr()
    w.fuse_w, w.fuse_b = P["fuse.weight"].data_ptr(), P["fuse.bias"].data_ptr()
    w.filt_uniform = packs.head_uniform_mask(P)
    keep += [dsn_w, dsn_b]
    return w, keep


def native_forward(P, packs, pool: ArenaPool, x: torch.Tensor, with_side_out: bool, keep: bool):
    _check_frame(x)
    for name in ("stages.0.0.weight", "fuse.weight"):
        if not P[name].is_cuda or P[name].dtype != torch.float32:
            raise RuntimeError("OSVOS_VGG parameters must be fp32 tensors on the GPU")
    x = x.contiguous().float()
    N, _, H, W = x.shape
    dev = x.device
    arena = pool.take(N, H, W, dev)
    ap, an = _aligned_ptr(arena)
    w, keep_alive = _weights_struct(P, packs)
    fused = torch.empty((N, 1, H, W), dtype=torch.float32, device=dev)
    outs = [torch.empty((N, 1, H, W), dtype=torch.float32, device=dev) for _ in range(4)] if with_side_out else None
    so = ptr_array4([o.data_ptr() for o in outs]) if with_side_out else None
    idx = dev.index if dev.index is not None else torch.cuda.current_device()
    t0 = ops._pb()
    opts = packs.options
    aux = (pool.aux_stream(idx) if N >= 2 and opts.fwd_aux and opts.two_streams and not packs.flags.forward_one_stream
           else 0)
    if aux:
        check(lib().fosvos_vgg_forward_streams(pool.ctx(idx), ctypes.byref(w), x.data_ptr(), N, H, W, ap, an, fused.data_ptr(),
                                               so, torch.cuda.current_stream(idx).cuda_stream, aux), "vgg_forward_streams")
    else:
        check(lib().fosvos_vgg_forward(ctypes.byref(w), x.data_ptr(), N, H, W, ap, an, fused.data_ptr(), so, idx,
                                       torch.cuda.current_stream(idx).cuda_stream), "vgg_forward")
    ops._pe(t0, "vgg_forward", 2.0 * 129.114e9 * N * H * W / (480 * 854), 0.0)
    if not keep:
        pool.give(N, H, W, arena)
        arena = None
    return (outs if outs is not None else [None] * 4) + [fused], (arena, x, w, keep_alive, (N, H, W))


def native_backward(P, packs, saved, d_outs, inplace: bool) -> Dict[str, torch.Tensor]:
    arena, x, w, keep_alive, (N, H, W) = saved
    dev = x.device
    d_fused = d_outs[4]
    d_so, with_so = _side_grads(d_outs)
    grads: Dict[str, torch.Tensor] = {}
    if d_fused is None and not with_so:
        return grads
    g = VggGrads()
    hold = []

    def slot(name: str) -> int:
        p = P[name]
        if inplace:
            if p.grad is None or p.grad.dtype != torch.float32 or not p.grad.is_contiguous():
                p.grad = torch.zeros_like(p, memory_format=torch.contiguous_format)
            torch.autograd.graph.increment_version(p.grad)
            return p.grad.data_ptr()
        t = torch.empty_like(p, memory_format=torch.contiguous_format)
        grads[name] = t
        return t.data_ptr()

    for c, (wn, bn) in enumerate(_CONV_NAMES):
        g.conv_w[c], g.conv_b[c] = slot(wn), slot(bn)
    for i in range(4):
        g.side_w[i], g.side_b[i] = slot(f"side_prep.{i}.weight"), slot(f"side_prep.{i}.bias")
    g.fuse_w, g.fuse_b = slot("fuse.weight"), slot("fuse.bias")
    dsn_tmp = None
    if with_so:
        dsn_tmp = (torch.zeros((4, 16), dtype=torch.float32, device=dev), torch.zeros((4,), dtype=torch.float32, device=dev))
        g.dsn_w, g.dsn_b = dsn_tmp[0].data_ptr(), dsn_tmp[1].data_ptr()
    flags = packs.flags
    overwrite = inplace and flags.overwrite_grads
    if overwrite and with_so:
        raise RuntimeError("OSVOS_VGG backward: overwrite_grads with side-output gradients (score_dsn accumulates through a scratch)")
    g.accumulate = 1 if inplace and not overwrite else 0
    idx = dev.index if dev.index is not None else torch.cuda.current_device()
    aux = packs.arenas.aux_stream(idx) if packs.options.two_streams else 0
    g.defer_join = 1 if (flags.defer_wgrad_join and inplace and aux) else 0
    g.bucket_events = 1 if flags.publish_grad_buckets else 0
    g.last_pass_of_cycle = 1 if flags.last_pass_of_cycle else 0
    if d_fused is not None:
        d_fused = d_fused.contiguous().float()
        hold.append(d_fused)
    dso = None
    if with_so:
        d_so = [t.contiguous().float() for t in d_so]
        hold += d_so
        dso = ptr_array4([t.data_ptr() for t in d_so])
    ap, an = _aligned_ptr(arena)
    t0 = ops._pb()
    check(lib().fosvos_vgg_backward(packs.arenas.ctx(idx), ctypes.byref(w), ctypes.byref(g), x.data_ptr(), N, H, W, ap, an,
                                    d_fused.data_ptr() if d_fused is not None else None, dso,
                                    torch.cuda.current_stream(idx).cuda_stream, aux or None),
          "vgg_backward")
    ops._pe(t0, "vgg_backward", 2.0 * (2 * 129.114e9 - 0.708e9) * N * H * W / (480 * 854), 0.0)
    if with_so:
        for i in range(4):
            gw, gb = dsn_tmp[0][i].reshape(1, 16, 1, 1), dsn_tmp[1][i:i + 1]
            if inplace:
                for name, val in ((f"score_dsn.{i}.weight", gw), (f"score_dsn.{i}.bias", gb)):
                    p = P[name]
                    if p.grad is None:
                        p.grad = val.clone()
                    else:
                        p.grad.add_(val)
            else:
                grads[f"score_dsn.{i}.weight"], grads[f"score_dsn.{i}.bias"] = gw.clone(), gb.clone()
    del hold, keep_alive
    if g.defer_join:
        packs.arenas.hold(N, H, W, arena, x)
    else:
        packs.arenas.give(N, H, W, arena)
    return grads


class _OSVOSFunction(torch.autograd.Function):

    @staticmethod
    def forward(ctx, packs: PackedWeights, with_side_out: bool, inplace: bool, x: torch.Tensor, *params: torch.Tensor):
        P = dict(zip(PARAM_NAMES, params))
        if USE_NATIVE_LOOP:
            outs, sv = native_forward(P, packs, packs.arenas, x, with_side_out, keep=True)
        else:
            outs, sv = forward(P, packs, x, with_side_out=with_side_out, keep=True)
        ctx.sv = sv
        ctx.packs = packs
        ctx.P = P
        ctx.set_materialize_grads(False)
        ctx.with_side_out = with_side_out
        ctx.inplace = inplace
        if not with_side_out:
            outs = [torch.empty(0, device=x.device) for _ in range(4)] + [outs[4]]
            ctx.mark_non_differentiable(*outs[:4])
        return tuple(outs)

    @staticmethod
    def backward(ctx, *d_outs):
        if ctx.sv is None:
            raise RuntimeError("OSVOS_VGG backward called but no activations were kept")
        d = list(d_outs)
        if not ctx.with_side_out:
            d = [None] * 4 + [d[4]]
        if USE_NATIVE_LOOP:
            grads = native_backward(ctx.P, ctx.packs, ctx.sv, d, inplace=ctx.inplace)
        else:
            grads = backward(ctx.P, ctx.packs, ctx.sv, d, inplace=ctx.inplace)
# ... 23 lines not shown
```

### fosvos_amd/fosvos_hip/ops.py

```python
from __future__ import annotations

from typing import List, Optional, Sequence, Tuple

import torch

from . import CONV_OUT_F32, CONV_RELU, check, int_array4, lib, ptr_array4

_BF16 = torch.bfloat16
_F32 = torch.float32


def _need(t: torch.Tensor, dtype, what: str) -> torch.Tensor:
    if not t.is_cuda:
        raise RuntimeError(f"{what}: tensor must live on the GPU (the HIP path has no CPU fallback)")
    if t.dtype != dtype:
        raise TypeError(f"{what}: expected {dtype}, got {t.dtype}")
    if not t.is_contiguous():
        raise ValueError(f"{what}: tensor must be contiguous")
    return t


def _ctx(t: torch.Tensor) -> Tuple[int, int]:
    dev = t.device.index if t.device.index is not None else torch.cuda.current_device()
    return dev, torch.cuda.current_stream(dev).cuda_stream
# ... 215 lines not shown
    import ctypes
    tiles, wgs = ctypes.c_int(), ctypes.c_int()
    check(lib().fosvos_conv3x3_first_plan(n, h, w, ctypes.byref(tiles), ctypes.byref(wgs)), "conv3x3_first_plan")
    return tiles.value, wgs.value


def conv3x3_fwd(x: torch.Tensor, w_packed: torch.Tensor, bias: Optional[torch.Tensor], ci: int, co: int,
                relu: bool = True, out_f32: bool = False) -> torch.Tensor:
    _need(x, _BF16, "conv3x3_fwd x"); _need(w_packed, _BF16, "conv3x3_fwd packed weight")
    n, h, wd, cx = x.shape
    if cx != _ru(ci, 32):
        raise ValueError(f"conv3x3_fwd: x has {cx} channels, expected {_ru(ci, 32)} (Ci={ci} padded to 32)")
    L = lib()
    if w_packed.numel() != L.fosvos_packed_weight_elems(co, ci):
        raise ValueError("conv3x3_fwd: packed weight size does not match (Co, Ci)")
    if bias is not None:
        _need(bias, _F32, "conv3x3_fwd bias")
        if bias.numel() != co:
            raise ValueError("conv3x3_fwd: bias size")
    y = torch.empty((n, h, wd, co), dtype=_F32 if out_f32 else _BF16, device=x.device)
    flags = (CONV_RELU if relu else 0) | (CONV_OUT_F32 if out_f32 else 0)
    ws, wsn = _WS.get(L.fosvos_conv3x3_workspace_bytes(n, h, wd, ci, co), x.device)
    dev, st = _ctx(x)
    t0 = _pb()
    check(L.fosvos_conv3x3_fwd(x.data_ptr(), w_packed.data_ptr(), _p(bias), y.data_ptr(), n, h, wd, ci, co, flags, ws, wsn,
                               dev, st), "conv3x3_fwd")
    _pe(t0, "conv3x3_fwd", 2.0 * n * h * wd * 9 * ci * co,
        n * h * wd * (2 * cx + (4 if out_f32 else 2) * co) + 2 * 9 * ci * co)
    return y


def conv3x3_fwd_pool(x: torch.Tensor, w_packed: torch.Tensor, bias: Optional[torch.Tensor], ci: int, co: int,
                     relu: bool = True) -> Tuple[torch.Tensor, torch.Tensor]:
    _need(x, _BF16, "conv3x3_fwd_pool x"); _need(w_packed, _BF16, "conv3x3_fwd_pool packed weight")
    n, h, wd, cx = x.shape
    if cx != _ru(ci, 32):
        raise ValueError(f"conv3x3_fwd_pool: x has {cx} channels, expected {_ru(ci, 32)}")
    L = lib()
    if w_packed.numel() != L.fosvos_packed_weight_elems(co, ci):
        raise ValueError("conv3x3_fwd_pool: packed weight size does not match (Co, Ci)")
    if bias is not None:
        _need(bias, _F32, "conv3x3_fwd_pool bias")
    y = torch.empty((n, h, wd, co), dtype=_BF16, device=x.device)
    yp = torch.empty((n, (h + 1) // 2, (wd + 1) // 2, co), dtype=_BF16, device=x.device)
    ws, wsn = _WS.get(L.fosvos_conv3x3_workspace_bytes(n, h, wd, ci, co), x.device)
    dev, st = _ctx(x)
    t0 = _pb()
    check(L.fosvos_conv3x3_fwd_pool(x.data_ptr(), w_packed.data_ptr(), _p(bias), y.data_ptr(), yp.data_ptr(), n, h, wd, ci,
                                    co, CONV_RELU if relu else 0, ws, wsn, dev, st), "conv3x3_fwd_pool")
    _pe(t0, "conv3x3_fwd", 2.0 * n * h * wd * 9 * ci * co, n * h * wd * (2 * cx + 2 * co) + 2 * 9 * ci * co + yp.numel() * 2)
    return y, yp


def conv3x3_dgrad(dy: torch.Tensor, w_dgrad_packed: torch.Tensor, ci: int, co: int,
                  relu_src: Optional[torch.Tensor] = None, addend: Optional[torch.Tensor] = None,
                  out: Optional[torch.Tensor] = None, relu_bits: Optional[torch.Tensor] = None) -> torch.Tensor:
    _need(dy, _BF16, "conv3x3_dgrad dy"); _need(w_dgrad_packed, _BF16, "conv3x3_dgrad packed weight")
    n, h, wd, cy = dy.shape
    if cy != _ru(co, 32):
        raise ValueError(f"conv3x3_dgrad: dy has {cy} channels, expected {_ru(co, 32)}")
    L = lib()
    if w_dgrad_packed.numel() != L.fosvos_packed_weight_elems(ci, co):
        raise ValueError("conv3x3_dgrad: packed weight size does not match (Ci, Co)")
    shape = (n, h, wd, ci)
    for t, nm in ((relu_src, "relu_src"), (addend, "addend"), (out, "out")):
        if t is not None:
            _need(t, _BF16, f"conv3x3_dgrad {nm}")
            if tuple(t.shape) != shape:
                raise ValueError(f"conv3x3_dgrad: {nm} shape {tuple(t.shape)} != {shape}")
    dx = out if out is not None else torch.empty(shape, dtype=_BF16, device=dy.device)
    ws, wsn = _WS.get(L.fosvos_conv3x3_workspace_bytes(n, h, wd, co, ci), dy.device)
    dev, st = _ctx(dy)
    t0 = _pb()
    if relu_bits is not None:
        if relu_src is not None or relu_bits.dtype != torch.uint8 or tuple(relu_bits.shape) != (n, h, wd, ci // 8) or \
                not relu_bits.is_contiguous() or not relu_bits.is_cuda:
            raise ValueError("conv3x3_dgrad: relu_bits must be a contiguous uint8 [N,H,W,Ci/8] GPU tensor, given instead of relu_src")
        check(L.fosvos_conv3x3_dgrad_bits(dy.data_ptr(), w_dgrad_packed.data_ptr(), relu_bits.data_ptr(), _p(addend),
                                          dx.data_ptr(), n, h, wd, ci, co, ws, wsn, dev, st), "conv3x3_dgrad_bits")
    else:
        check(L.fosvos_conv3x3_dgrad(dy.data_ptr(), w_dgrad_packed.data_ptr(), _p(relu_src), _p(addend), dx.data_ptr(), n, h, wd,
                                     ci, co, ws, wsn, dev, st), "conv3x3_dgrad")
    _pe(t0, "conv3x3_dgrad", 2.0 * n * h * wd * 9 * ci * co,
        n * h * wd * 2 * (cy + ci * (1 + (relu_src is not None) + (addend is not None))) + 2 * 9 * ci * co)
    return dx


def conv3x3_dgrad_unpool(dy: torch.Tensor, w_dgrad_packed: torch.Tensor, ci: int, co: int, x: torch.Tensor,
                         d_pooled: torch.Tensor, out: Optional[torch.Tensor] = None) -> torch.Tensor:
    _need(dy, _BF16, "conv3x3_dgrad_unpool dy"); _need(w_dgrad_packed, _BF16, "conv3x3_dgrad_unpool packed weight")
    _need(x, _BF16, "conv3x3_dgrad_unpool x"); _need(d_pooled, _BF16, "conv3x3_dgrad_unpool d_pooled")
    n, h, wd, cy = dy.shape
    if cy != _ru(co, 32):
        raise ValueError(f"conv3x3_dgrad_unpool: dy has {cy} channels, expected {_ru(co, 32)}")
    L = lib()
    if w_dgrad_packed.numel() != L.fosvos_packed_weight_elems(ci, co):
        raise ValueError("conv3x3_dgrad_unpool: packed weight size does not match (Ci, Co)")
    if tuple(x.shape) != (n, h, wd, ci) or tuple(d_pooled.shape) != (n, (h + 1) // 2, (wd + 1) // 2, ci):
        raise ValueError(f"conv3x3_dgrad_unpool: x {tuple(x.shape)} / d_pooled {tuple(d_pooled.shape)} do not match "
                         f"{(n, h, wd, ci)} and its ceil-mode pooled map")
    if out is not None:
        _need(out, _BF16, "conv3x3_dgrad_unpool out")
        if tuple(out.shape) != (n, h, wd, ci) or out.data_ptr() == x.data_ptr():
            raise ValueError("conv3x3_dgrad_unpool: out must have x's shape and must not alias it")
    dx = out if out is not None else torch.empty((n, h, wd, ci), dtype=_BF16, device=dy.device)
    ws, wsn = _WS.get(L.fosvos_conv3x3_workspace_bytes(n, h, wd, co, ci), dy.device)
# ... 20 lines not shown
        if accumulate:
            raise ValueError("conv3x3_wgrad: accumulate needs an existing db")
        db = torch.empty((co,), dtype=_F32, device=x.device)
    _need(dw, _F32, "conv3x3_wgrad dw")
    ws, wsn = _WS.get(L.fosvos_conv3x3_wgrad_workspace_bytes(n, h, wd, ci, co), x.device)
    dev, st = _ctx(x)
    t0 = _pb()
    check(L.fosvos_conv3x3_wgrad_slabs(x.data_ptr(), dy.data_ptr(), 1 if with_bias else 0, n, h, wd, ci, co, ws, wsn, dev, st),
          "conv3x3_wgrad_slabs")
    _pe(t0, "conv3x3_wgrad", 2.0 * n * h * wd * 9 * ci * co, n * h * wd * 2 * (ci + dy.shape[3]))
    t0 = _pb()
    check(L.fosvos_conv3x3_wgrad_reduce(dw.data_ptr(), _p(db) if with_bias else None, n, h, wd, ci, co,
                                        1 if accumulate else 0, ws, wsn, dev, st), "conv3x3_wgrad_reduce")
    _pe(t0, "wgrad_reduce", 0.0, 4 * 9 * ci * co * 3)
    return dw, (db if with_bias else None)


def conv3x3_wgrad_one_call(x: torch.Tensor, dy: torch.Tensor, ci: int, co: int, with_bias: bool = True):
    _need(x, _BF16, "conv3x3_wgrad x"); _need(dy, _BF16, "conv3x3_wgrad dy")
    n, h, wd, _ = x.shape
    L = lib()
    dw = torch.empty((co, ci, 3, 3), dtype=_F32, device=x.device)
    db = torch.empty((co,), dtype=_F32, device=x.device) if with_bias else None
    ws, wsn = _WS.get(L.fosvos_conv3x3_wgrad_workspace_bytes(n, h, wd, ci, co), x.device)
    dev, st = _ctx(x)
    check(L.fosvos_conv3x3_wgrad(x.data_ptr(), dy.data_ptr(), dw.data_ptr(), _p(db), n, h, wd, ci, co, 0, ws, wsn, dev, st),
          "conv3x3_wgrad")
    return dw, db


def maxpool_fwd(x: torch.Tensor) -> torch.Tensor:
    _need(x, _BF16, "maxpool_fwd")
    n, h, w, c = x.shape
    y = torch.empty((n, (h + 1) // 2, (w + 1) // 2, c), dtype=_BF16, device=x.device)
    dev, st = _ctx(x)
    t0 = _pb()
    check(lib().fosvos_maxpool2x2_ceil_fwd(x.data_ptr(), y.data_ptr(), n, h, w, c, dev, st), "maxpool2x2_ceil_fwd")
    _pe(t0, "maxpool_fwd", 0.0, 2 * (x.numel() + y.numel()))
    return y


def maxpool_bwd(x: torch.Tensor, dy: torch.Tensor, relu_mask: bool = True) -> torch.Tensor:
    _need(x, _BF16, "maxpool_bwd x"); _need(dy, _BF16, "maxpool_bwd dy")
    n, h, w, c = x.shape
    if tuple(dy.shape) != (n, (h + 1) // 2, (w + 1) // 2, c):
        raise ValueError("maxpool_bwd: dy shape mismatch")
    dx = torch.empty_like(x)
    dev, st = _ctx(x)
    t0 = _pb()
    check(lib().fosvos_maxpool2x2_ceil_bwd(x.data_ptr(), dy.data_ptr(), dx.data_ptr(), n, h, w, c, 1 if relu_mask else 0,
                                           dev, st), "maxpool2x2_ceil_bwd")
    _pe(t0, "maxpool_bwd", 0.0, 2 * (2 * x.numel() + dy.numel()))
    return dx


def head_fwd(side: Sequence[torch.Tensor], filt: Sequence[torch.Tensor], filt1: Optional[Sequence[torch.Tensor]],
             dsn_w: Optional[torch.Tensor], dsn_b: Optional[torch.Tensor], fuse_w: torch.Tensor, fuse_b: torch.Tensor,
             H: int, W: int, with_side_out: bool = True, filt_uniform: int = 0):
    n = side[0].shape[0]
    for s in range(4):
        _need(side[s], _F32, "head_fwd side"); _need(filt[s], _F32, "head_fwd filt")
        k = 4 << s
        if side[s].shape[3] != 16 or tuple(filt[s].shape) != (k, k, 16):
            raise ValueError("head_fwd: side/filter shape")
    _need(fuse_w, _F32, "head_fwd fuse_w"); _need(fuse_b, _F32, "head_fwd fuse_b")
    dev_t = side[0].device
    fused = torch.empty((n, 1, H, W), dtype=_F32, device=dev_t)
    outs = None
    so_ptrs = [None] * 4
    f1_ptrs = [None] * 4
    if with_side_out:
        outs = [torch.empty((n, 1, H, W), dtype=_F32, device=dev_t) for _ in range(4)]
        so_ptrs = [o.data_ptr() for o in outs]
        for s in range(4):
            _need(filt1[s], _F32, "head_fwd filt1")
        f1_ptrs = [f.data_ptr() for f in filt1]
        _need(dsn_w, _F32, "head_fwd dsn_w"); _need(dsn_b, _F32, "head_fwd dsn_b")
    dev, st = _ctx(side[0])
    t0 = _pb()
    check(lib().fosvos_head_fwd(ptr_array4([t.data_ptr() for t in side]), int_array4([t.shape[1] for t in side]),
                                int_array4([t.shape[2] for t in side]), ptr_array4([t.data_ptr() for t in filt]),
                                ptr_array4(f1_ptrs), _p(dsn_w) if with_side_out else None,
                                _p(dsn_b) if with_side_out else None, fuse_w.data_ptr(), fuse_b.data_ptr(),
                                fused.data_ptr(), ptr_array4(so_ptrs), n, H, W, int(filt_uniform) & 15, dev, st), "head_fwd")
    _pe(t0, "head_fwd", 2.0 * n * H * W * 256, 4 * (sum(t.numel() for t in side) + n * H * W * (5 if with_side_out else 1)))
    return fused, outs


def filters_uniform_mask(filt: Sequence[torch.Tensor]) -> int:
    mask = 0
    for s, f in enumerate(filt):
        if bool((f == f[..., :1]).all().item()):
            mask |= 1 << s
    return mask


def head_bwd(side: Sequence[torch.Tensor], filt: Sequence[torch.Tensor], filt1: Optional[Sequence[torch.Tensor]],
             dsn_w: Optional[torch.Tensor], fuse_w: torch.Tensor, d_fused: Optional[torch.Tensor],
             d_side_out: Optional[Sequence[torch.Tensor]], H: int, W: int, filt_uniform: int = 0):
    n = side[0].shape[0]
    dev_t = side[0].device
    with_so = d_side_out is not None
    if d_fused is not None:
        _need(d_fused, _F32, "head_bwd d_fused")
    d_side = [torch.empty((n, t.shape[1], t.shape[2], 32), dtype=_BF16, device=dev_t) for t in side]
    d_fuse_w = torch.empty((64,), dtype=_F32, device=dev_t)
# ... 1199 lines not shown
```

### fosvos_amd/networks/osvos_vgg.py

```python
import dataclasses
import os
from copy import deepcopy

import torch
import torch.nn as nn
import torch.nn.modules as modules

from fosvos_hip import engine
from layers.osvos_layers import interp_surgery
from util.logger import get_logger

log = get_logger(__file__)


class OSVOS_VGG(nn.Module):
    def __init__(self, pretrained=1):
        super(OSVOS_VGG, self).__init__()
        lay_list = [[64, 64],
                    ['M', 128, 128],
                    ['M', 256, 256, 256],
                    ['M', 512, 512, 512],
                    ['M', 512, 512, 512]]
        in_channels = [3, 64, 128, 256, 512]

# ... 122 lines not shown
            elif isinstance(m, nn.ConvTranspose2d):
                m.weight.data.zero_()
                m.weight.data = interp_surgery(m)

        if pretrained == 1:
            self._load_from_pytorch()
        elif pretrained == 2:
            self._load_from_caffe()

    def _load_from_pytorch(self):
        log.info('Loading weights from PyTorch VGG')
        try:
            from torchvision.models import vgg16
        except ImportError as e:
            raise RuntimeError("OSVOS_VGG(pretrained=1) copies torchvision's ImageNet VGG-16, which needs "
                               "torchvision and network access; use pretrained=0 + load_state_dict, or "
                               "pretrained=2 with vgg_hed_caffe.mat") from e
        _vgg = vgg16(pretrained=True)
        src = [m for m in _vgg.features if isinstance(m, nn.Conv2d)]
        dst = [m for stage in self.stages for m in stage if isinstance(m, nn.Conv2d)]
        for d, s in zip(dst, src):
            d.weight = deepcopy(s.weight)
            d.bias = deepcopy(s.bias)

    def _load_from_caffe(self):
        log.info('Loading weights from Caffe VGG')
        import scipy.io
        from config.mypath import Path
        caffe_weights = scipy.io.loadmat(os.path.join(Path.models_dir(), 'vgg_hed_caffe.mat'))
        convs = [m for stage in self.stages for m in stage if isinstance(m, nn.Conv2d)]
        for k, conv in enumerate(convs):
            c_w = torch.from_numpy(caffe_weights['weights'][0][k].transpose())
            c_b = torch.from_numpy(caffe_weights['biases'][0][k][:, 0])
            assert conv.weight.data.shape == c_w.shape
            assert conv.bias.data.shape == c_b.shape
            conv.weight.data = c_w
            conv.bias.data = c_b


def _pass_flag(name):
    def get(self):
        return getattr(self._packs.flags, name)

    def set_(self, value):
        if name == 'defer_wgrad_join' and not value:
            self._packs.arenas.join()
        setattr(self._packs.flags, name, bool(value))

    return property(get, set_, doc='engine.PassFlags.' + name)


for _field in dataclasses.fields(engine.PassFlags):
    setattr(OSVOS_VGG, _field.name, _pass_flag(_field.name))
```

### fosvos_amd/train_offline.py

```python
import timeit
from pathlib import Path
from typing import Optional

import torch
from torch import optim

from config.mypath import Path as P
from fosvos_hip.engine import PassFlags
from fosvos_hip.options import LoopOptions
from layers.osvos_layers import (class_balanced_cross_entropy_loss, class_balanced_cross_entropy_loss_frames_multi,
                                 stage_frames_loss_multi)
from util import gpu_handler, io_helper, experiment_helper, args_helper
from util.logger import get_logger
from util.network_provider import NetworkProvider, provider_mapping
from util.settings import OfflineSettings
import parallel

log = get_logger(__file__)
_hip_cbce = class_balanced_cross_entropy_loss

save_dir_models = Path('models')
save_dir_results = Path('results')
db_root_dir = None
synthetic_size = None
# ... 23 lines not shown
            net_provider.load_network_test()
        data_loader = io_helper.get_data_loader_test(db_root_dir, settings.batch_size_test, synthetic=synthetic_size)
        if settings.variant_offline is None:
            save_dir = save_dir_results / net_provider.name / 'offline'
        else:
            save_dir = save_dir_results / net_provider.name / str(settings.variant_offline) / 'offline'
        experiment_helper.test(net_provider, data_loader, save_dir, settings.is_visualizing_results,
                               settings.eval_speeds)


def _get_summary_writer():
    return io_helper.get_summary_writer(save_dir_models, comment='-offline')


def _losses(net, minibatch):
    inputs, gts = gpu_handler.cast_cuda_if_possible([minibatch['image'], minibatch['gt']])
    outputs = net.forward(inputs)
    counts = parallel.batch_label_counts(gts) if data_parallel else None
    return [class_balanced_cross_entropy_loss(o, gts, size_average=False, batch_counts=counts) for o in outputs]


def window_closes(n_window: int, counter_gradient: int, avg_grad_every_n: int, max_window: int, end_of_epoch: bool) -> bool:
    return ((counter_gradient + n_window) % avg_grad_every_n == 0) or n_window >= max_window or end_of_epoch


def plan_passes(shapes, group: int):
    buckets = {}
    for i, shape in enumerate(shapes):
        shape = tuple(int(v) for v in shape)
        alone = shape[0] != 1 or (shape[-2] * shape[-1]) % 4 != 0
        buckets.setdefault(('alone', i) if alone else shape, []).append(i)
    passes = []
    for key, idx in buckets.items():
        if key[0] == 'alone':
            passes.append((idx, False))
        else:
            passes.extend((idx[j:j + group], True) for j in range(0, len(idx), group))
    return passes


def _losses_frames(outputs, gts, map_scale, ones, staged=None):
    k = gts.shape[0]
    if gts.is_cuda and class_balanced_cross_entropy_loss is _hip_cbce:
        return class_balanced_cross_entropy_loss_frames_multi(outputs, gts, map_scale, size_average=False,
                                                              backward_seed=(ones, 1.0), staged=staged), ones[:k]
    losses = torch.stack([torch.stack([class_balanced_cross_entropy_loss(o[i:i + 1], gts[i:i + 1], size_average=False)
                                       for o in outputs]) for i in range(k)])
    return losses, torch.tensor(map_scale, dtype=losses.dtype, device=losses.device).expand(k, -1)


def _train(net_provider: NetworkProvider, data_loader_train, data_loader_test, optimizer: optim.SGD, summary_writer,
           start_epoch: int, n_epochs: int, avg_grad_every_n: int, snapshot_every_n: int,
           is_testing_while_training: bool, test_every_n: int, *, options: Optional[LoopOptions] = None,
           microbatch_group: int = 1) -> dict:
    if options is None:
        options = LoopOptions.from_env()
    microbatch_group = int(microbatch_group)
    if microbatch_group < 1:
        raise ValueError('microbatch_group must be at least 1, got {}'.format(microbatch_group))
    if microbatch_group > 1 and data_parallel:
        raise ValueError('microbatch_group > 1 with data_parallel: that mode splits every BATCH over the ranks with class '
                         'counts of the whole batch; a grouped pass keeps the counts per frame')
    log.info('Start of offline training')
    net = net_provider.network
    flags = getattr(net, 'pass_flags', None) or PassFlags()
    world = parallel.world_size() if data_parallel else 1
    local_accum = avg_grad_every_n
    named = list(net.named_parameters())
    flat = parallel.FlatGrads.attach(net, [p for _, p in named], names=[n for n, _ in named])
    sync = parallel.GradSync(net, flat, options)
    device = next(net.parameters()).device

    n_samples_train = len(data_loader_train)
    loss_train, loss_test, losses_train = [], [], []
    counter_gradient = 0
    n_iters = 0
    n_passes = 0
    max_window = max(microbatch_group, options.group_window)
    ones = torch.ones((microbatch_group, 5), device=device) if microbatch_group > 1 else None
    reserved_frames = getattr(net, 'reserve_arena_frames', None)

    def log_epoch(epoch, running, n_images, start_time):
        if world > 1:
            torch.distributed.all_reduce(running, op=torch.distributed.ReduceOp.SUM)
        vals = (running / n_samples_train).tolist()
        loss_train.append(vals[-1])
        losses_train.append(vals)
        summary_writer.add_scalar('data/total_loss_epoch', vals[-1], epoch)
        log.info('[Epoch: %d, numImages: %5d]' % (epoch, n_images))
        for l in range(len(vals)):
            log.info('Loss %d: %f' % (l, vals[l]))
        log.info('Execution time: ' + str(timeit.default_timer() - start_time))

    def step_if_due():
        nonlocal counter_gradient
        if counter_gradient % local_accum == 0:
            net.join_gradients()
            sync.finish()
            optimizer.step()
            flat.zero()
            counter_gradient = 0

    def run_window(window, epoch, running):
        nonlocal counter_gradient, n_iters, n_passes
        w = 1 - epoch / n_epochs
        map_scale = [w / avg_grad_every_n] * 4 + [1.0 / avg_grad_every_n]
        for idx, batched in plan_passes([mb['image'].shape for mb in window], microbatch_group):
            if not batched:
                losses = _losses(net, window[idx[0]])
                running += torch.stack([l.detach() for l in losses])
                loss = w * sum(losses[:-1]) + losses[-1]
                loss.backward(torch.full_like(loss.detach(), 1.0 / avg_grad_every_n))
            else:
                if len(idx) == 1:
                    inputs, gts = window[idx[0]]['image'], window[idx[0]]['gt']
                else:
                    inputs = torch.cat([window[i]['image'] for i in idx])
                    gts = torch.cat([window[i]['gt'] for i in idx])
                inputs, gts = gpu_handler.cast_cuda_if_possible([inputs, gts])
                staged = None
                if options.stage_loss and gts.is_cuda and class_balanced_cross_entropy_loss is _hip_cbce:
                    staged = stage_frames_loss_multi(gts.contiguous().float(), 5)
                    if staged is not None:
                        gts = staged.label
                outputs = net.forward(inputs)
                losses, seed = _losses_frames(outputs, gts, map_scale, ones, staged)
                losses.backward(seed)
                if staged is not None:
                    staged.finish()
                running += losses.detach().sum(0)
            counter_gradient += len(idx)
            n_iters += len(idx)
            n_passes += 1
        step_if_due()

    time_all_start = timeit.default_timer()
    net.accumulate_grads_in_place = True
    if microbatch_group > 1 and reserved_frames is not None:
        net.reserve_arena_frames = min(microbatch_group, avg_grad_every_n)
    if not options.defer_join:
        net.join_gradients()
    flags.defer_wgrad_join = options.defer_join
    try:
        for epoch in range(start_epoch, n_epochs):
            start_time = timeit.default_timer()
            sampler = getattr(data_loader_train, 'sampler', None)
            if hasattr(sampler, 'set_epoch'):
                sampler.set_epoch(epoch)
            running = torch.zeros(5, device=device)
            window = []
            for index, minibatch in enumerate(data_loader_train):
                if microbatch_group > 1:
                    end_of_epoch = index % n_samples_train == n_samples_train - 1
                    window.append(minibatch)
                    if window_closes(len(window), counter_gradient, local_accum, max_window, end_of_epoch):
                        run_window(window, epoch, running)
                        window = []
                    if end_of_epoch:
                        log_epoch(epoch, running, index + 1, start_time)
                    continue
                losses = _losses(net, minibatch)
                running += torch.stack([l.detach() for l in losses])
                loss = (1 - epoch / n_epochs) * sum(losses[:-1]) + losses[-1]

                if index % n_samples_train == n_samples_train - 1:
                    log_epoch(epoch, running, index + 1, start_time)

                last_of_cycle = world > 1 and (counter_gradient + 1) % local_accum == 0
                if last_of_cycle:
                    sync.arm()
                loss.backward(torch.full_like(loss.detach(), 1.0 / avg_grad_every_n))
                if last_of_cycle:
                    sync.begin()
                counter_gradient += 1
                n_iters += 1
                n_passes += 1
                step_if_due()
            if window:
                run_window(window, epoch, running)

            if (epoch % snapshot_every_n) == snapshot_every_n - 1 and epoch != 0 and parallel.rank() == 0:
                net_provider.save_model(epoch)

            if is_testing_while_training and epoch % test_every_n == (test_every_n - 1):
                with torch.no_grad():
                    running_t = torch.zeros(5, device=device)
                    for index, minibatch in enumerate(data_loader_test):
                        running_t += torch.stack(_losses(net, minibatch))
                    vals = (running_t / max(len(data_loader_test), 1)).tolist()
                loss_test.append(vals[-1])
                summary_writer.add_scalar('data/test_loss_epoch', vals[-1], epoch)
                for l in range(len(vals)):
                    log.info('***Testing *** Loss %d: %f' % (l, vals[l]))
        summary_writer.close()
    finally:
        net.join_gradients()
        flags.defer_wgrad_join = False
        if microbatch_group > 1 and reserved_frames is not None:
            net.reserve_arena_frames = reserved_frames
    if torch.cuda.is_available():
        torch.cuda.synchronize()
    return {'loss_train': loss_train, 'loss_test': loss_test, 'losses_train': losses_train, 'iterations': n_iters,
            'passes': n_passes, 'seconds': timeit.default_timer() - time_all_start}


def main(argv=None):
    global db_root_dir, synthetic_size, data_parallel, resident_train_set, microbatch_group
    args = args_helper.parse_args(is_online=False, argv=argv)
    if args.network != 'vgg16':
        raise SystemExit('only --network vgg16 is implemented on the HIP path (ResNet family: SURVEY.md §8 f4)')
    data_parallel = bool(args.data_parallel) and parallel.init_distributed()
    gpu_handler.select_gpu(args.gpu_id)
    db_root_dir = P.db_root_dir()
    synthetic_size = (args.height, args.width) if args.synthetic else None
    resident_train_set = bool(args.resident_train_set)
    microbatch_group = args.microbatch_group
    save_dir_models.mkdir(parents=True, exist_ok=True)
    save_dir_results.mkdir(parents=True, exist_ok=True)

    settings = OfflineSettings(is_training=args.is_training, is_testing=args.is_testing, start_epoch=0,
                               n_epochs=args.n_epochs or 240, avg_grad_every_n=args.avg_grad_every_n or 10,
                               snapshot_every_n=40, is_testing_while_training=False, test_every_n=5,
                               batch_size_train=1, batch_size_test=1, is_visualizing_network=False,
                               is_visualizing_results=False, is_loading_vgg_caffe=False,
                               variant_offline=args.variant_offline, eval_speeds=args.eval_speeds)
    provider_class = provider_mapping[('offline', args.network)]
    net_provider = provider_class(args.network, save_dir_models, settings, variant_offline=args.variant_offline)
    if args.synthetic:
        log.warning('--synthetic: starting from OSVOS_VGG(pretrained=0) random init')
        net_provider.load_network_train = lambda: net_provider.init_network(pretrained=0)
    train_and_test(net_provider, settings)


if __name__ == '__main__':
    main()
```

### fosvos_amd/train_online.py

```python
import timeit
from pathlib import Path
from typing import Optional

import numpy as np
import torch
from torch import optim

from config.mypath import Path as P
from fosvos_hip.engine import PassFlags
from fosvos_hip.options import LoopOptions
from layers.osvos_layers import class_balanced_cross_entropy_loss, class_balanced_cross_entropy_loss_frames, stage_frames_loss
from util import gpu_handler, io_helper, experiment_helper, args_helper
from util.logger import get_logger
from util.network_provider import NetworkProvider, provider_mapping
from util.settings import OnlineSettings
import parallel

log = get_logger(__file__)
_hip_cbce = class_balanced_cross_entropy_loss

save_dir_models = Path('models')
save_dir_results = Path('results')
path_stem = 'vgg16/online'
db_root_dir = None
# ... 211 lines not shown
        while self.pending:
            items, landed, slots = self.pending[0]
            if block:
                for ev in landed:
                    ev.synchronize()
            elif not all(ev.query() for ev in landed):
                break
            self.pending.pop(0)
            for ep, mb, host_vals, i in items:
                self.running_host += float(host_vals[i])
                if ep % self.log_every == self.log_every - 1:
                    value = self.running_host / self.n_samples
                    self.running_host = 0.0
                    self.loss_tr.append(value)
                    log.info('[Epoch {0}: {1}, numImages: {2}]'.format(self.seq_name, ep + 1, mb + 1))
                    log.info('Loss {0}: {1}'.format(self.seq_name, value))
                    self.summary_writer.add_scalar('data/total_loss_epoch', value, ep)
            self.ring_free.extend(slots)

    def record(self, group, losses) -> None:
        frames = [(g[0], g[1]) for g in group]
        if self.ring is not None:
            if not self.ring_free:
                self.flush(True)
            if not self.ring_free:
                self.window.append((frames, losses.to('cpu'), _Landed(), None))
                return
            slot = self.ring_free.pop()
            host_vals = self.ring[slot, :len(frames)]
            host_vals.copy_(losses, non_blocking=True)
            landed = torch.cuda.Event()
            landed.record()
        else:
            slot, host_vals, landed = None, losses.clone(), _Landed()
        self.window.append((frames, host_vals, landed, slot))

    def close_window(self) -> None:
        if not self.window:
            return
        items = sorted(((ep, mb, host_vals, i) for frames, host_vals, _, _ in self.window
                        for i, (ep, mb) in enumerate(frames)), key=lambda t: (t[0], t[1]))
        slots = [slot for _, _, _, slot in self.window if slot is not None]
        self.pending.append((items, [landed for _, _, landed, _ in self.window], slots))
        self.window.clear()
        self.flush(False)


def _get_summary_writer(seq_name: str):
    return io_helper.get_summary_writer(Path('tensorboard') / path_stem)


def _train(net_provider: NetworkProvider, dataloader, optimizer: optim.SGD, summary_writer, seq_name: str,
           start_epoch: int, n_epochs: int, avg_grad_every_n: int, snapshot_every_n: int, *,
           options: Optional[LoopOptions] = None) -> dict:
    if options is None:
        options = LoopOptions.from_env()
    log.info('Start of Online Training, sequence: ' + seq_name)
    net = net_provider.network
    flags = getattr(net, 'pass_flags', None)
    native = flags is not None and all(callable(getattr(net, f, None)) for f in ('wait_grad_bucket', 'join_gradients'))
    if flags is None:
        flags = PassFlags()
    world = parallel.world_size() if data_parallel else 1
    dp_on = data_parallel and parallel.collectives_on()
    local_accum = parallel.split_accumulation(avg_grad_every_n, world)
    flat = parallel.FlatGrads.attach_module(net)
    sync = parallel.GradSync(net, flat, options)
    on_gpu = flat.flat.is_cuda and native

    early_buckets = [b for b, bid in enumerate(flat.bucket_ids) if bid < parallel.VGG_EARLY_BUCKETS]
    late_buckets = [b for b in range(len(flat.slices)) if b not in early_buckets]
    split_step = (on_gpu and bool(early_buckets) and bool(late_buckets)
                  and getattr(net, 'publishes_grad_buckets', True)
                  and hasattr(optimizer, '_tables') and options.split_step)
    early_params = [p for b in early_buckets for p in flat.bucket_params[b]]
    early_ids = {id(p) for p in early_params}
    late_params = [p for group in optimizer.param_groups for p in group['params'] if id(p) not in early_ids]
    early_prefixes = tuple(pre for b in early_buckets for pre in parallel.VGG_BUCKETS[flat.bucket_ids[b]])

    lazy_zero = on_gpu and options.grad_overwrite
    grads_stale = False
    pass_streams = None
    if flat.flat.is_cuda:
        from fosvos_hip import engine as _engine
        dev_index = flat.flat.device.index if flat.flat.device.index is not None else torch.cuda.current_device()
        _engine.shared_stream(dev_index, "comm")
        if native and options.defer_join and options.pass_streams:
            pass_streams = [None, _engine.shared_stream(dev_index, "pass")]
    counter_gradient = 0
    log_every = max(n_epochs // 20, 1)
    device = next(net.parameters()).device
    max_group = options.microbatch_group
    max_window = max(max_group, options.group_window)
    consts = flat.cache.get(('online', avg_grad_every_n, max_group, str(device)))
    if consts is None:
        consts = flat.cache[('online', avg_grad_every_n, max_group, str(device))] = {
            'inv_avg': torch.ones((), device=device) / avg_grad_every_n,
            'inv_avg_k': torch.full((max_group,), 1.0 / avg_grad_every_n, device=device),
            'ring': torch.empty((64, max_group), dtype=torch.float32).pin_memory() if device.type == 'cuda' else None}
    inv_avg, inv_avg_k = consts['inv_avg'], consts['inv_avg_k']
    loss_log = _LossLog(consts['ring'], len(dataloader), log_every, seq_name, summary_writer)

    def is_snapshot_epoch(epoch: int) -> bool:
        return (epoch % snapshot_every_n) == snapshot_every_n - 1

    side_stream_used = False
    last_pass_on_side = False
# ... 74 lines not shown
                net.prepack_weights(early_prefixes)
                wait_side_stream()
                net.join_gradients()
                sync.finish()
                optimizer.step(only=late_params, tag='late', zero_grad=not lazy_zero)
            else:
                wait_side_stream()
                net.join_gradients()
                sync.finish()
                optimizer.step()
                if not lazy_zero:
                    flat.zero()
            grads_stale = lazy_zero
            counter_gradient = 0

    def run_window(window) -> None:
        nonlocal grads_stale
        buckets = {}
        for item in window:
            shape = tuple(item[2]['image'].shape)
            buckets.setdefault(shape if shape[0] == 1 else ('batch', id(item)), []).append(item)
        groups = [items[i:i + max_group] for items in buckets.values() for i in range(0, len(items), max_group)]
        multi = pass_streams is not None and not dp_on and len(groups) > 1 and max(len(g) for g in groups) <= 2
        if lazy_zero:
            whole_cycle = counter_gradient == 0 and len(groups) == 1 and len(groups[0]) == local_accum
            flags.overwrite_grads = whole_cycle
            if counter_gradient == 0:
                if grads_stale and not whole_cycle:
                    flat.zero()
                grads_stale = False
        if multi:
            net.prepack_weights()
            pass_streams[1].wait_stream(torch.cuda.current_stream(device))
        flags.forward_one_stream = multi
        for i, group in enumerate(groups):
            run_group(group, pass_streams[(len(groups) - 1 - i) % 2] if multi else None)
        if multi:
            wait_side_stream()
        loss_log.close_window()
        epoch, _idx, _mb, end_of_epoch = window[-1]
        if end_of_epoch and is_snapshot_epoch(epoch) and parallel.rank() == 0:
            net_provider.save_model(epoch, sequence=seq_name)

    time_all_start = timeit.default_timer()
    n_iters = 0
    if native:
        net.reserve_arena_frames = min(max_group, avg_grad_every_n)
    net.accumulate_grads_in_place = True
    net.compute_side_outputs = False
    if not options.defer_join:
        net.join_gradients()
    flags.defer_wgrad_join = options.defer_join
    try:
        window = []
        for epoch in range(start_epoch, n_epochs):
            n_mb = len(dataloader)
            for minibatch_index, minibatch in enumerate(dataloader):
                end_of_epoch = minibatch_index == n_mb - 1
                window.append((epoch, minibatch_index, minibatch, end_of_epoch))
                closes_cycle = (counter_gradient + len(window)) % local_accum == 0
                if closes_cycle or len(window) >= max_window or (end_of_epoch and is_snapshot_epoch(epoch)):
                    run_window(window)
                    window = []
        if window:
            run_window(window)
    finally:
        net.join_gradients()
        flags.defer_wgrad_join = False
        flags.publish_grad_buckets = False
        if lazy_zero:
            flags.overwrite_grads = False
            if grads_stale:
                flat.zero()
        flags.forward_one_stream = False
        net.compute_side_outputs = True
    time_enqueued = timeit.default_timer() - time_all_start
    if torch.cuda.is_available():
        torch.cuda.synchronize()
    loss_log.flush(True)
    time_for_all = timeit.default_timer() - time_all_start
    n_images = len(dataloader)
    log.info('Train {0}: total time {1} sec'.format(seq_name, str(time_for_all)))
    log.info('Train {0}: {1} images'.format(seq_name, str(n_images)))
    log.info('Train {0}: time per sample {1} sec'.format(seq_name, str(time_for_all / max(n_images, 1))))
    return {'loss': loss_log.loss_tr, 'seconds': time_for_all, 'iterations': n_iters, 'seconds_host_enqueue': time_enqueued,
            'comm_timing': sync.timing_summary() if sync.active and sync.timing else None}


def main(argv=None):
    global db_root_dir, synthetic_size, data_parallel, save_dir_models, save_dir_results, score, fast_test, png_fitted, device_decode
    global multi_object, synthetic_objects, clean, adapt
    args = args_helper.parse_args(is_online=True, argv=argv)
    if args.score and args.eval_speeds:
        raise SystemExit('--score needs the PNG-writing test pass; --eval-speeds writes nothing')
    if args.fast_test and args.eval_speeds:
        raise SystemExit('--fast-test is the PNG-writing test pass; --eval-speeds writes nothing')
    score = bool(args.score)
    fast_test = bool(args.fast_test)
    png_fitted = bool(args.png_fitted)
    device_decode = bool(args.device_decode)
    multi_object = bool(args.multi_object)
    clean = None
    if args.clean_min_area is not None or args.clean_largest or args.clean_temporal is not None:
        from fosvos_hip.options import CleanOptions
        clean = CleanOptions(min_area=args.clean_min_area or 0, largest=bool(args.clean_largest),
                             temporal_radius=args.clean_temporal)
    adapt = args.adapt
    synthetic_objects = int(args.objects)
    del scored_sequences[:]
    if args.network != 'vgg16':
        raise SystemExit('only --network vgg16 is implemented on the HIP path (ResNet family: SURVEY.md §8 f4)')
    data_parallel = bool(args.data_parallel) and parallel.init_distributed()
    gpu_handler.select_gpu(args.gpu_id)

    db_root_dir = P.db_root_dir()
    synthetic_size = (args.height, args.width) if args.synthetic else None
    save_dir_models.mkdir(parents=True, exist_ok=True)
    save_dir_results.mkdir(parents=True, exist_ok=True)
    path_input_model = Path(args.parent_model) if args.parent_model else save_dir_models / 'vgg16_epoch-239.pth'
    path_output_model_base = save_dir_models / path_stem
    path_output_model_base.mkdir(parents=True, exist_ok=True)

    settings = OnlineSettings(is_training=args.is_training, is_testing=args.is_testing, start_epoch=0,
                              n_epochs=args.n_epochs or 10000, avg_grad_every_n=args.avg_grad_every_n or 5,
                              snapshot_every_n=args.n_epochs or 10000, is_testing_while_training=False, test_every_n=5,
                              batch_size_train=1, batch_size_test=1, is_visualizing_network=False,
                              is_visualizing_results=False, offline_epoch=240, variant_offline=args.variant_offline,
# ... 55 lines not shown
```

### include/fosvos_hip.h

```cpp
#ifndef FOSVOS_HIP_H
#define FOSVOS_HIP_H

#include <stddef.h>
#include <stdint.h>

#ifdef __cplusplus
extern "C" {
#endif

#define FOSVOS_ABI_VERSION 33

#define FOSVOS_OK 0
#define FOSVOS_E_SHAPE (-1)
#define FOSVOS_E_ARG (-2)
#define FOSVOS_E_WORKSPACE (-3)
#define FOSVOS_E_HIP (-4)

#define FOSVOS_CONV_RELU 1u
#define FOSVOS_CONV_OUT_F32 2u
#define FOSVOS_CONV_FP32_MATH 4u

int fosvos_abi_version(void);

typedef struct fosvos_profile_record {
// ... 11 lines not shown
int fosvos_ctx_create(int device, fosvos_ctx **ctx_out);
int fosvos_ctx_destroy(fosvos_ctx *ctx);
int fosvos_ctx_device(const fosvos_ctx *ctx);

int fosvos_nchw_f32_to_nhwc_bf16(const float *src, uint16_t *dst, int N, int C, int H, int W, int Cpad,
                                 int device, void *stream);
int fosvos_nhwc_bf16_to_nchw_f32(const uint16_t *src, float *dst, int N, int C, int H, int W, int Cpad,
                                 int device, void *stream);
int fosvos_nhwc_f32_to_nchw_f32(const float *src, float *dst, int N, int C, int H, int W, int device, void *stream);
int fosvos_nchw_f32_to_nhwc_f32(const float *src, float *dst, int N, int C, int H, int W, int device, void *stream);
typedef struct fosvos_vgg_arena_layout_info {
    size_t total;
    int stage_h[5], stage_w[5];
    size_t act[13], gact[13], act_bytes[13];
    size_t pooled[4], gpooled[4], pooled_bytes[4];
    size_t side[4], side_bytes[4];
    size_t dside[4], dside_bytes[4];
    size_t bits0, bits0_bytes;
    size_t ws, ws_bytes, hws, hws_bytes;
    size_t wsa_conv[13], wsa_conv_bytes[13], wsa_side[4], wsa_side_bytes[4];
} fosvos_vgg_arena_layout_info;
int fosvos_vgg_arena_layout(int N, int H, int W, fosvos_vgg_arena_layout_info *out);

int fosvos_pack_conv3x3_weights(const float *w_oihw, int Co, int Ci, uint16_t *w_fwd, uint16_t *w_dgrad,
                                int device, void *stream);
size_t fosvos_packed_weight_elems(int out_ch, int in_ch);

typedef struct fosvos_pack_entry {
    const float *w;
    uint16_t *w_fwd, *w_dgrad;
    int Co, Ci;
} fosvos_pack_entry;
int fosvos_pack_conv3x3_weights_multi(const fosvos_pack_entry *entries, int n, int device, void *stream);

int fosvos_conv3x3_first_fwd(const float *frame, const float *w_oihw, const float *bias, uint16_t *y, uint8_t *relu_bits,
                             int N, int H, int W, int Co, int device, void *stream);
int fosvos_conv3x3_first_plan(int N, int H, int W, int *tiles, int *workgroups);
int fosvos_conv3x3_first_wgrad(const float *frame, const uint16_t *dy, float *dw_oihw, float *dbias, int N, int H,
                               int W, int Co, void *workspace, size_t workspace_bytes, int device, void *stream);
size_t fosvos_conv3x3_first_wgrad_workspace_bytes(int N, int H, int W, int Co);

int fosvos_conv3x3_fwd(const uint16_t *x, const uint16_t *w_packed, const float *bias, void *y, int N, int H, int W,
                       int Ci, int Co, unsigned flags, void *workspace, size_t workspace_bytes, int device,
                       void *stream);

int fosvos_conv3x3_s2_fwd(const uint16_t *x, const uint16_t *w_packed, const float *bias, uint16_t *y, int N, int H, int W,
                          int Ci, int Co, unsigned flags, void *workspace, size_t workspace_bytes, int device, void *stream);
int fosvos_conv3x3_fwd_add(const uint16_t *x, const uint16_t *w_packed, const float *bias, const uint16_t *addend,
                           void *y, int N, int H, int W, int Ci, int Co, unsigned flags, void *workspace,
                           size_t workspace_bytes, int device, void *stream);
int fosvos_conv3x3_fwd_pool(const uint16_t *x, const uint16_t *w_packed, const float *bias, uint16_t *y,
                            uint16_t *y_pool, int N, int H, int W, int Ci, int Co, unsigned flags, void *workspace,
                            size_t workspace_bytes, int device, void *stream);
size_t fosvos_conv3x3_workspace_bytes(int N, int H, int W, int in_ch, int out_ch);
typedef struct fosvos_conv3x3_plan_info {
    int tile_h, tile_w, tile_co;
    int k_splits;
    int workgroups;
    int persistent;
} fosvos_conv3x3_plan_info;
int fosvos_conv3x3_plan(int N, int H, int W, int in_ch, int out_ch, fosvos_conv3x3_plan_info *out);
int fosvos_conv3x3_fwd_plan(int N, int H, int W, int in_ch, int out_ch, unsigned flags, fosvos_conv3x3_plan_info *out);
int fosvos_conv3x3_dgrad(const uint16_t *dy, const uint16_t *w_dgrad_packed, const uint16_t *relu_src,
                         const uint16_t *addend, uint16_t *dx, int N, int H, int W, int Ci, int Co, void *workspace,
                         size_t workspace_bytes, int device, void *stream);
int fosvos_conv3x3_dgrad_bits(const uint16_t *dy, const uint16_t *w_dgrad_packed, const uint8_t *relu_bits,
                              const uint16_t *addend, uint16_t *dx, int N, int H, int W, int Ci, int Co, void *workspace,
                              size_t workspace_bytes, int device, void *stream);
int fosvos_conv3x3_dgrad_unpool(const uint16_t *dy, const uint16_t *w_dgrad_packed, const uint16_t *x,
                                const uint16_t *d_pooled, uint16_t *dx, int N, int H, int W, int Ci, int Co,
                                void *workspace, size_t workspace_bytes, int device, void *stream);
int fosvos_conv3x3_wgrad(const uint16_t *x, const uint16_t *dy, float *dw_oihw, float *dbias, int N, int H, int W,
                         int Ci, int Co, int accumulate, void *workspace, size_t workspace_bytes, int device,
                         void *stream);
size_t fosvos_conv3x3_wgrad_workspace_bytes(int N, int H, int W, int Ci, int Co);
int fosvos_conv3x3_wgrad_slabs(const uint16_t *x, const uint16_t *dy, int with_bias, int N, int H, int W, int Ci, int Co,
                               void *workspace, size_t workspace_bytes, int device, void *stream);
int fosvos_conv3x3_wgrad_reduce(float *dw_oihw, float *dbias, int N, int H, int W, int Ci, int Co, int accumulate,
                                void *workspace, size_t workspace_bytes, int device, void *stream);

int fosvos_maxpool2x2_ceil_fwd(const uint16_t *x, uint16_t *y, int N, int H, int W, int C, int device, void *stream);
int fosvos_maxpool2x2_ceil_bwd(const uint16_t *x, const uint16_t *dy, uint16_t *dx, int N, int H, int W, int C,
                               int relu_mask, int device, void *stream);

int fosvos_head_fwd(const float *const side[4], const int hs[4], const int ws[4], const float *const filt[4],
                    const float *const filt1[4], const float *dsn_w , const float *dsn_b ,
                    const float *fuse_w , const float *fuse_b , float *fused,
                    float *const side_out[4] , int N, int H, int W, int filt_uniform, int device,
                    void *stream);
int fosvos_head_bwd(const float *const side[4], const int hs[4], const int ws[4], const float *const filt[4],
                    const float *const filt1[4], const float *dsn_w, const float *fuse_w, const float *d_fused,
                    const float *const d_side_out[4], uint16_t *const d_side[4], float *d_fuse_w, float *d_fuse_b,
                    float *d_dsn_w, float *d_dsn_b, int N, int H, int W, int filt_uniform ,
                    void *workspace, size_t workspace_bytes, int device, void *stream);
size_t fosvos_head_bwd_workspace_bytes(int N, int H, int W);

int fosvos_cbce_loss(const float *logits, const float *label, int64_t numel, int size_average, float grad_scale,
                     float *loss_out, float *grad, void *workspace, size_t workspace_bytes, int device,
                     void *stream);
size_t fosvos_cbce_workspace_bytes(int64_t numel);
int fosvos_cbce_loss_frames(const float *logits, const float *label, int64_t frame_numel, int n_frames, int size_average,
                            float grad_scale, float *loss_out, float *grad, void *workspace, size_t workspace_bytes,
                            int device, void *stream);
#define FOSVOS_CBCE_COUNT 1
#define FOSVOS_CBCE_LOSS 2
#define FOSVOS_CBCE_FINISH 4
int fosvos_cbce_loss_frames_parts(const float *logits, const float *label, int64_t frame_numel, int n_frames,
                                  int size_average, float grad_scale, float *loss_out, float *grad, void *workspace,
                                  size_t workspace_bytes, int parts, int device, void *stream);
#define FOSVOS_CBCE_MAX_MAPS 8
size_t fosvos_cbce_multi_workspace_bytes(int64_t frame_numel, int n_frames, int n_maps);
int fosvos_cbce_loss_frames_multi(const float *const *logits, const float *label, int64_t frame_numel, int n_frames,
                                  int n_maps, int size_average, const float *map_scale, float *loss_out, float *const *grad,
                                  void *workspace, size_t workspace_bytes, int parts, int device, void *stream);
int fosvos_cbce_loss_batch_counts(const float *logits, const float *label, int64_t numel, int size_average,
                                  float grad_scale, const double *batch_counts, float *loss_out, float *grad,
                                  void *workspace, size_t workspace_bytes, int device, void *stream);
size_t fosvos_cbce_void_workspace_bytes(int64_t frame_numel, int n_frames);
int fosvos_cbce_loss_frames_void(const float *logits, const float *label, const uint8_t *void_px, int64_t frame_numel,
                                 int n_frames, int size_average, float grad_scale, float *loss_out, float *grad,
                                 void *workspace, size_t workspace_bytes, int device, void *stream);

#define FOSVOS_SGD_FIRST_STEP 1
#define FOSVOS_SGD_ZERO_GRAD 2
typedef struct fosvos_sgd_entry {
    float *param;
    const float *grad;
    float *momentum_buf;
    int64_t numel;
    float lr;
    float weight_decay;
} fosvos_sgd_entry;
int fosvos_sgd_momentum_step(const fosvos_sgd_entry *table, int n_tensors, int64_t max_numel, float momentum,
                             int first_step, int device, void *stream);

int fosvos_augment_sample(const uint8_t *frame, const uint8_t *mask, int H, int W, int flip, const int32_t *col_taps,
// ... 114 lines not shown
    const fosvos_resnet_block *blocks;
    fosvos_conv2d_desc side[4];
    const float *filt[4];
    const float *filt1[4];
    int stride[4];
    const float *dsn_w, *dsn_b, *fuse_b;
} fosvos_resnet_net;
size_t fosvos_resnet_arena_bytes(const fosvos_resnet_net *net, int N, int H, int W);
int fosvos_resnet_forward(const fosvos_resnet_net *net, const float *frame, int N, int H, int W, void *arena,
                          size_t arena_bytes, float *fused, float *const side_out[4], int device, void *stream,
                          fosvos_ctx *ctx, void *aux_stream);

typedef struct fosvos_vgg_weights {
    const float *conv_w[13];
    const float *conv_b[13];
    const uint16_t *conv_wf[13];
    const uint16_t *conv_wd[13];
    const float *side_b[4];
    const uint16_t *side_wf[4];
    const uint16_t *side_wd[4];
    const float *filt[4];
    const float *filt1[4];
    const float *dsn_w;
    const float *dsn_b;
    const float *fuse_w;
    const float *fuse_b;
    int filt_uniform;
} fosvos_vgg_weights;

typedef struct fosvos_vgg_grads {
    float *conv_w[13];
    float *conv_b[13];
    float *side_w[4];
    float *side_b[4];
    float *dsn_w;
    float *dsn_b;
    float *fuse_w;
    float *fuse_b;
    int accumulate;
    int defer_join;
    int bucket_events;
    int last_pass_of_cycle;
} fosvos_vgg_grads;

size_t fosvos_vgg_arena_bytes(int N, int H, int W);
int fosvos_vgg_forward(const fosvos_vgg_weights *w, const float *frame, int N, int H, int W, void *arena,
                       size_t arena_bytes, float *fused, float *const side_out[4], int device, void *stream);
int fosvos_vgg_forward_streams(fosvos_ctx *ctx, const fosvos_vgg_weights *w, const float *frame, int N, int H, int W,
                               void *arena, size_t arena_bytes, float *fused, float *const side_out[4], void *stream,
                               void *aux_stream);
int fosvos_vgg_backward(fosvos_ctx *ctx, const fosvos_vgg_weights *w, const fosvos_vgg_grads *g, const float *frame, int N,
                        int H, int W, void *arena, size_t arena_bytes, const float *d_fused,
                        const float *const d_side_out[4], void *stream, void *aux_stream);
int fosvos_vgg_grad_bucket_wait(fosvos_ctx *ctx, int bucket, void *stream);

#ifdef __cplusplus
}
#endif
#endif
```

Measured before the change: 1250 frames/s.

## Store stage-1 pool winner codes instead of dense conv1_2 activation

Adds a fused conv3x3+ReLU+maxpool variant of the persistent kernel that writes only the pooled map and a 4-bit argmax code per element. It no longer writes the full-resolution stage-1 activation. A new pool backward kernel routes gradients by those codes instead of re-reading the dense activation. The aim is to cut HBM writes and reads of the largest activation in forward and backward. In exchange it adds code-generation ALU work in the epilogue and a new flag path through the forward and backward passes, and its correctness depends on tie-breaking matching the old maxpool.

```diff
diff --git a/fosvos_amd/csrc/common.hpp b/fosvos_amd/csrc/common.hpp
--- a/fosvos_amd/csrc/common.hpp
+++ b/fosvos_amd/csrc/common.hpp
@@ -121,7 +121,9 @@
 int conv_pp_workgroups();
 int conv_pp_forward(const uint16_t *x, const uint16_t *w_packed, const float *bias, uint16_t *y, uint16_t *y_pool, int N,
                     int H, int W, int Cin_pad, int Cout, int Co_pad, bool relu, hipStream_t st,
-                    const uint8_t *mask_bits = nullptr);
+                    const uint8_t *mask_bits = nullptr, uint32_t *codes = nullptr);
+
+bool conv3x3_pool_codes_applicable(int N, int H, int W, int Ci, int Co);
 
 inline int64_t cdiv(int64_t a, int64_t b) { return (a + b - 1) / b; }
 inline int roundup(int a, int b) { return (a + b - 1) / b * b; }
diff --git a/fosvos_amd/csrc/conv_igemm.hip b/fosvos_amd/csrc/conv_igemm.hip
--- a/fosvos_amd/csrc/conv_igemm.hip
+++ b/fosvos_amd/csrc/conv_igemm.hip
@@ -899,6 +899,36 @@
     return dispatch(a, Ci, workspace, workspace_bytes, (hipStream_t)stream);
 }
 
+namespace fosvos {
+bool conv3x3_pool_codes_applicable(int N, int H, int W, int Ci, int Co) {
+    if (N <= 0 || H <= 0 || W <= 0 || Ci <= 0 || Co <= 0 || Co % 64 != 0) return false;
+    if ((int64_t)H * W * roundup(Ci, 32) * 2 >= 0x7fffffffLL || (int64_t)H * W * Co * 4 >= 0x7fffffffLL) return false;
+    return forward_takes_pp(N, H, W, Ci, Co, FOSVOS_CONV_RELU);
+}
+}
+
+extern "C" size_t fosvos_conv3x3_pool_codes_bytes(int N, int H, int W, int C) {
+    if (N <= 0 || H <= 0 || W <= 0 || C <= 0 || C % 8 != 0) return 0;
+    return (size_t)N * ((H + 1) / 2) * ((W + 1) / 2) * (C / 8) * 4;
+}
+
+extern "C" int fosvos_conv3x3_fwd_pool_codes(const uint16_t *x, const uint16_t *w_packed, const float *bias,
+                                             uint16_t *y_pool, uint32_t *codes, int N, int H, int W, int Ci, int Co,
+                                             unsigned flags, int device, void *stream) {
+    if (int rc = check_common(x, w_packed, y_pool, N, H, W, Ci, Co, "conv3x3_fwd_pool_codes")) return rc;
+    FOSVOS_REQUIRE(codes, FOSVOS_E_ARG, "conv3x3_fwd_pool_codes: null codes output");
+    FOSVOS_REQUIRE(((uintptr_t)codes & 3) == 0, FOSVOS_E_ARG, "conv3x3_fwd_pool_codes: codes must be 4-byte aligned");
+    FOSVOS_REQUIRE(flags == FOSVOS_CONV_RELU, FOSVOS_E_ARG,
+                   "conv3x3_fwd_pool_codes: flags 0x%x (the codes are taken on post-ReLU values: FOSVOS_CONV_RELU)", flags);
+    FOSVOS_REQUIRE(Co % 64 == 0, FOSVOS_E_SHAPE, "conv3x3_fwd_pool_codes: Co=%d must be a multiple of 64", Co);
+    FOSVOS_REQUIRE(conv3x3_pool_codes_applicable(N, H, W, Ci, Co), FOSVOS_E_SHAPE,
+                   "conv3x3_fwd_pool_codes: N=%d H=%d W=%d Ci=%d Co=%d is not a shape of the persistent kernel (use "
+                   "fosvos_conv3x3_fwd_pool)", N, H, W, Ci, Co);
+    FOSVOS_ENTER(device);
+    return conv_pp_forward(x, w_packed, bias, nullptr, y_pool, N, H, W, roundup(Ci, 32), Co, roundup(Co, 16), true,
+                           (hipStream_t)stream, nullptr, codes);
+}
+
 extern "C" int fosvos_conv3x3_dgrad_bits(const uint16_t *dy, const uint16_t *w_dgrad_packed, const uint8_t *relu_bits,
                                          const uint16_t *addend, uint16_t *dx, int N, int H, int W, int Ci, int Co,
                                          void *workspace, size_t workspace_bytes, int device, void *stream) {
diff --git a/fosvos_amd/csrc/conv_pp.hip b/fosvos_amd/csrc/conv_pp.hip
--- a/fosvos_amd/csrc/conv_pp.hip
+++ b/fosvos_amd/csrc/conv_pp.hip
@@ -22,6 +22,7 @@
     const float *bias;
     uint16_t *y;
     uint16_t *y_pool;
+    uint32_t *codes;
     const uint8_t *mask_bits;
     int N, H, W, Cin, Cout, Co_pad;
     int tiles_x, tiles_y, n_tiles;
@@ -89,7 +90,28 @@
     __device__ __forceinline__ int x0() const { return tx * TW; }
 };
 
-template <bool RELU, bool POOL, bool MASK = false>
+__device__ __forceinline__ unsigned pool_code_word(const uint4 &a, const uint4 &b, const uint4 &c, const uint4 &d, uint4 &m) {
+    const unsigned av[4] = {a.x, a.y, a.z, a.w}, bv[4] = {b.x, b.y, b.z, b.w}, cv[4] = {c.x, c.y, c.z, c.w},
+                   dv[4] = {d.x, d.y, d.z, d.w};
+    unsigned mv[4], code = 0;
+#pragma unroll
+    for (int i = 0; i < 4; ++i) {
+        auto sub = [](unsigned p, unsigned q) {
+            return __builtin_bit_cast(unsigned, __builtin_bit_cast(fosvos_i16x2, p) - __builtin_bit_cast(fosvos_i16x2, q));
+        };
+        const unsigned m1 = max_nonneg_bf16x2(av[i], bv[i]), m2 = max_nonneg_bf16x2(m1, cv[i]);
+        mv[i] = max_nonneg_bf16x2(m2, dv[i]);
+        const unsigned s1 = sub(av[i], bv[i]), s2 = sub(m1, cv[i]), s3 = sub(m2, dv[i]);
+        const unsigned pm = sub(0u, mv[i]) & 0x80008000u;
+        const unsigned n3 = s3 & pm, n2 = s2 & ~s3 & pm, n1 = s1 & ~(s2 | s3) & pm, n0 = ~(s1 | s2 | s3) & pm;
+        const unsigned r = n3 | (n2 >> 1) | (n1 >> 2) | (n0 >> 3);
+        code = (code >> 4) | r;
+    }
+    m = make_uint4(mv[0], mv[1], mv[2], mv[3]);
+    return code;
+}
+
+template <bool RELU, bool POOL, bool MASK = false, bool CODES = false>
 __global__ __launch_bounds__(NT) __attribute__((amdgpu_waves_per_eu(2, 2))) void k_conv3x3_pp(const Args a) {
     extern __shared__ __attribute__((aligned(16))) char smem_pp[];
     const unsigned lds0 = __builtin_amdgcn_readfirstlane((unsigned)(size_t)(lds_void *)smem_pp);
@@ -249,6 +271,7 @@
     auto store_slot = [&](int slot) {
         if (!st_pending) return;
         if (slot < 4) {
+            if constexpr (CODES) return;
             const auto y_rsrc = __builtin_amdgcn_make_buffer_rsrc(a.y + (int64_t)dn_n * H * W * Cout, 0, H * W * Cout * 2, 0x00020000);
             const int gy = dn_y0 + 2 * wm + (slot >> 1), gx = dn_x0 + (slot & 1) * 16 + cl;
             const unsigned off = (gy < H && gx < W) ? (unsigned)(((gy * W + gx) * Cout + n0 + kq * 8) * 2) : 0x80000000u;
@@ -263,6 +286,46 @@
             const int ih = slot - 4;
             const int OH = (H + 1) >> 1, OW = (W + 1) >> 1;
             const bool edge = dn_y0 + TH > H || dn_x0 + TW > W;
+            if constexpr (CODES) {
+                const int jp = cl & 1;
+                const auto c_rsrc = __builtin_amdgcn_make_buffer_rsrc(a.codes + (int64_t)dn_n * OH * OW * (Cout >> 3), 0,
+                                                                      OH * OW * (Cout >> 3) * 4, 0x00020000);
+                const auto pc_rsrc = __builtin_amdgcn_make_buffer_rsrc(a.y_pool + (int64_t)dn_n * OH * OW * Cout, 0,
+                                                                       OH * OW * Cout * 2, 0x00020000);
+                const int oy = (dn_y0 >> 1) + wm, ox = (dn_x0 >> 1) + ih * 8 + (cl >> 1);
+                const bool ok = oy < OH && ox < OW;
+                const int px = oy * OW + ox;
+                uint4 t[2] = {pk[ih][0], pk[ih][1]}, bo[2] = {pk[ih + 2][0], pk[ih + 2][1]};
+                if (edge) {
+                    const int gy = dn_y0 + 2 * wm, gx = dn_x0 + ih * 16 + cl;
+                    if (!(gy < H && gx < W)) t[0] = t[1] = make_uint4(0, 0, 0, 0);
+                    if (!(gy + 1 < H && gx < W)) bo[0] = bo[1] = make_uint4(0, 0, 0, 0);
+                }
+                auto pick = [&](const uint4 &v0, const uint4 &v1, bool second) {
+                    const unsigned s0[4] = {v0.x, v0.y, v0.z, v0.w}, s1[4] = {v1.x, v1.y, v1.z, v1.w};
+                    unsigned o[4];
+#pragma unroll
+                    for (int q = 0; q < 4; ++q) {
+                        if (!second) {
+                            const unsigned nb = (unsigned)__builtin_amdgcn_update_dpp(0, (int)s1[q], 0xA0, 0xF, 0xF, true);
+                            o[q] = jp ? nb : s0[q];
+                        } else {
+                            const unsigned nb = (unsigned)__builtin_amdgcn_update_dpp(0, (int)s0[q], 0xF5, 0xF, 0xF, true);
+                            o[q] = jp ? s1[q] : nb;
+                        }
+                    }
+                    return make_uint4(o[0], o[1], o[2], o[3]);
+                };
+                const uint4 pa = pick(t[0], t[1], false), pb = pick(t[0], t[1], true);
+                const uint4 pcx = pick(bo[0], bo[1], false), pd = pick(bo[0], bo[1], true);
+                uint4 m;
+                const unsigned code = pool_code_word(pa, pb, pcx, pd, m);
+                const unsigned poff = ok ? (unsigned)((px * Cout + n0 + kq * 8 + jp * 32) * 2) : 0x80000000u;
+                const unsigned coff = ok ? (unsigned)((px * (Cout >> 3) + (n0 >> 3) + kq + jp * 4) * 4) : 0x80000000u;
+                __builtin_amdgcn_raw_buffer_store_b128(__builtin_bit_cast(u32x4, m), pc_rsrc, poff, 0, 0);
+                __builtin_amdgcn_raw_buffer_store_b32(code, c_rsrc, coff, 0, 0);
+                return;
+            }
             const auto p_rsrc = __builtin_amdgcn_make_buffer_rsrc(a.y_pool + (int64_t)dn_n * OH * OW * Cout, 0,
                                                                   OH * OW * Cout * 2, 0x00020000);
             const int oy = (dn_y0 >> 1) + wm, ox = (dn_x0 >> 1) + ih * 8 + (cl >> 1);
@@ -395,11 +458,14 @@
 
 
 int conv_pp_forward(const uint16_t *x, const uint16_t *w_packed, const float *bias, uint16_t *y, uint16_t *y_pool, int N,
-                    int H, int W, int Cin_pad, int Cout, int Co_pad, bool relu, hipStream_t st, const uint8_t *mask_bits) {
+                    int H, int W, int Cin_pad, int Cout, int Co_pad, bool relu, hipStream_t st, const uint8_t *mask_bits,
+                    uint32_t *codes) {
+    FOSVOS_REQUIRE(!codes || (y_pool && !y && !mask_bits), FOSVOS_E_ARG,
+                   "conv3x3 (persistent): winner codes go with the pooled map, without the dense one");
     FOSVOS_REQUIRE(!y_pool || relu, FOSVOS_E_ARG, "conv3x3 (persistent): the fused pool takes post-ReLU values");
     FOSVOS_REQUIRE(!mask_bits || (!relu && !y_pool && !bias), FOSVOS_E_ARG, "conv3x3 (persistent): the bit mask is the data gradient's epilogue");
     pp::Args a{};
-    a.x = x; a.w = w_packed; a.bias = bias; a.y = y; a.y_pool = y_pool; a.mask_bits = mask_bits;
+    a.x = x; a.w = w_packed; a.bias = bias; a.y = y; a.y_pool = y_pool; a.mask_bits = mask_bits; a.codes = codes;
     a.N = N; a.H = H; a.W = W; a.Cin = Cin_pad; a.Cout = Cout; a.Co_pad = Co_pad;
     a.tiles_x = (int)cdiv(W, pp::TW);
     a.tiles_y = (int)cdiv(H, pp::TH);
@@ -410,10 +476,11 @@
     a.stamps = g_pp_stamps;
 #endif
     void (*kern)(const pp::Args) = mask_bits ? pp::k_conv3x3_pp<false, false, true>
+                                   : codes   ? pp::k_conv3x3_pp<true, true, false, true>
                                    : y_pool  ? pp::k_conv3x3_pp<true, true>
                                    : relu    ? pp::k_conv3x3_pp<true, false> : pp::k_conv3x3_pp<false, false>;
-    const int which = mask_bits ? 3 : y_pool ? 2 : relu ? 1 : 0;
-    static bool once[64][4];
+    const int which = mask_bits ? 3 : codes ? 4 : y_pool ? 2 : relu ? 1 : 0;
+    static bool once[64][5];
     int dev = 0;
     FOSVOS_HIP_CHECK(hipGetDevice(&dev));
     if (dev >= 0 && dev < 64 && !once[dev][which]) {
@@ -421,7 +488,8 @@
                                              pp::LDS_BYTES));
         once[dev][which] = true;
     }
-    FOSVOS_PROF(mask_bits ? "k_conv3x3_pp<false, false, true>" : y_pool ? "k_conv3x3_pp<true, true, false>"
+    FOSVOS_PROF(mask_bits ? "k_conv3x3_pp<false, false, true>" : codes ? "k_conv3x3_pp<true, true, false, true>"
+                : y_pool  ? "k_conv3x3_pp<true, true, false>"
                 : relu    ? "k_conv3x3_pp<true, false, false>" : "k_conv3x3_pp<false, false, false>", st,
                 2.0 * N * H * W * 9.0 * Cin_pad * Cout);
     hipLaunchKernelGGL(kern, dim3(conv_pp_workgroups()), dim3(pp::NT), pp::LDS_BYTES, st, a);
diff --git a/fosvos_amd/csrc/pool.hip b/fosvos_amd/csrc/pool.hip
--- a/fosvos_amd/csrc/pool.hip
+++ b/fosvos_amd/csrc/pool.hip
@@ -82,6 +82,33 @@
     if (vx && vy) *reinterpret_cast<uint4 *>(dxn + o11) = repack8(r3);
 }
 
+__global__ __launch_bounds__(256) void k_pool_bwd_codes(const uint32_t *__restrict__ codes, const uint16_t *__restrict__ dy,
+                                                         uint16_t *__restrict__ dx, int H, int W, int C, int OH, int OW) {
+    const int groups = C >> 3;
+    const int col = blockIdx.x * 256 + threadIdx.x;
+    if (col >= OW * groups) return;
+    const int ox = col / groups, g = col - ox * groups;
+    const int oy = blockIdx.y;
+    const int64_t n = blockIdx.z;
+    uint16_t *dxn = dx + n * H * W * C;
+    const int iy = oy * 2, ix = ox * 2;
+    const bool vx = ix + 1 < W, vy = iy + 1 < H;
+    const int o00 = (iy * W + ix) * C + g * 8;
+    const int o01 = o00 + C, o10 = o00 + W * C, o11 = o10 + C;
+    const int64_t p = (n * OH + oy) * OW + ox;
+    const uint4 gv = *reinterpret_cast<const uint4 *>(dy + p * C + g * 8);
+    const uint32_t code = codes[p * groups + g];
+    auto routed = [&](int k) {
+        const uint32_t c = code >> k;
+        return make_uint4(gv.x & ((c & 0x00010001u) * 0xffffu), gv.y & (((c >> 4) & 0x00010001u) * 0xffffu),
+                          gv.z & (((c >> 8) & 0x00010001u) * 0xffffu), gv.w & (((c >> 12) & 0x00010001u) * 0xffffu));
+    };
+    *reinterpret_cast<uint4 *>(dxn + o00) = routed(0);
+    if (vx) *reinterpret_cast<uint4 *>(dxn + o01) = routed(1);
+    if (vy) *reinterpret_cast<uint4 *>(dxn + o10) = routed(2);
+    if (vx && vy) *reinterpret_cast<uint4 *>(dxn + o11) = routed(3);
+}
+
 inline int grid_for(int64_t total) {
     int64_t g = cdiv(total, 256);
     if (g > 16384) g = 16384;
@@ -119,3 +146,19 @@
     FOSVOS_LAUNCH_CHECK();
     return FOSVOS_OK;
 }
+
+extern "C" int fosvos_maxpool2x2_ceil_bwd_codes(const uint32_t *codes, const uint16_t *dy, uint16_t *dx, int N, int H, int W,
+                                                int C, int device, void *stream) {
+    FOSVOS_REQUIRE(codes && dy && dx, FOSVOS_E_ARG, "maxpool_bwd_codes: null pointer");
+    FOSVOS_REQUIRE(N > 0 && H > 0 && W > 0 && C > 0 && C % 8 == 0, FOSVOS_E_SHAPE,
+                   "maxpool_bwd_codes: bad shape N=%d H=%d W=%d C=%d (C %% 8 must be 0)", N, H, W, C);
+    const int OH = (H + 1) / 2, OW = (W + 1) / 2;
+    FOSVOS_REQUIRE((int64_t)H * W * C < 0x7fffffffLL && OH <= 65535 && N <= 65535, FOSVOS_E_SHAPE,
+                   "maxpool_bwd_codes: image too large (N=%d H=%d W=%d C=%d)", N, H, W, C);
+    FOSVOS_ENTER(device);
+    FOSVOS_PROF("k_pool_bwd_codes", stream, 0.0);
+    hipLaunchKernelGGL(k_pool_bwd_codes, dim3((unsigned)cdiv((int64_t)OW * (C / 8), 256), (unsigned)OH, (unsigned)N), dim3(256), 0,
+                       (hipStream_t)stream, codes, dy, dx, H, W, C, OH, OW);
+    FOSVOS_LAUNCH_CHECK();
+    return FOSVOS_OK;
+}
diff --git a/fosvos_amd/csrc/vgg_net.hip b/fosvos_amd/csrc/vgg_net.hip
--- a/fosvos_amd/csrc/vgg_net.hip
+++ b/fosvos_amd/csrc/vgg_net.hip
@@ -94,6 +94,21 @@
         if (rc_ != FOSVOS_OK) return rc_; \
     } while (0)
 
+bool fwd_split_on() {
+    static const bool on = lab_env_int("FOSVOS_FWD_SPLIT", 1) != 0;
+    return on;
+}
+
+bool stage1_compact(unsigned flags, int N, int H, int W) {
+    if (!(flags & FOSVOS_VGG_COMPACT_STAGE1) || N <= 0 || H <= 0 || W <= 0) return false;
+    if (fwd_split_on() && N >= 2) {
+        const int na = (N + 1) / 2;
+        return conv3x3_pool_codes_applicable(na, H, W, kCin[1], kCout[1]) &&
+               conv3x3_pool_codes_applicable(N - na, H, W, kCin[1], kCout[1]);
+    }
+    return conv3x3_pool_codes_applicable(N, H, W, kCin[1], kCout[1]);
+}
+
 int check_net(const void *w, const void *frame, const void *arena, int N, int H, int W, size_t arena_bytes,
               const Arena &a, const char *who) {
     FOSVOS_REQUIRE(w && frame && arena, FOSVOS_E_ARG, "%s: null pointer", who);
@@ -145,19 +160,24 @@
 
 namespace {
 int forward_impl(hipEvent_t *ev, const fosvos_vgg_weights *w, const float *frame, int N, int H, int W, void *arena,
-                 size_t arena_bytes, float *fused, float *const side_out[4], int device, void *stream, void *aux_stream) {
+                 size_t arena_bytes, float *fused, float *const side_out[4], int device, void *stream, void *aux_stream,
+                 unsigned flags) {
     const Arena a = make_arena(N, H, W);
     FOSVOS_TRY(check_net(w, frame, arena, N, H, W, arena_bytes, a, "vgg_forward"));
     FOSVOS_REQUIRE(fused, FOSVOS_E_ARG, "vgg_forward: null output");
+    FOSVOS_REQUIRE((flags & ~FOSVOS_VGG_COMPACT_STAGE1) == 0, FOSVOS_E_ARG, "vgg_forward: unknown flags 0x%x", flags);
+    const bool compact = stage1_compact(flags, N, H, W);
     char *base = reinterpret_cast<char *>(arena);
+    auto codes1 = [&](int f0) {
+        return reinterpret_cast<uint32_t *>(base + a.act[1]) + (size_t)f0 * a.sh[1] * a.sw[1] * (kCout[1] / 8);
+    };
     auto act = [&](int c) { return reinterpret_cast<uint16_t *>(base + a.act[c]); };
     void *ws = base + a.ws;
     hipStream_t sm = (hipStream_t)stream;
     const bool par = ev != nullptr && aux_stream != nullptr && aux_stream != stream;
     hipStream_t sa = par ? (hipStream_t)aux_stream : sm;
     if (par) FOSVOS_ENTER(device);
-    static const bool split_on = lab_env_int("FOSVOS_FWD_SPLIT", 1) != 0;
-    if (split_on && N >= 2) {
+    if (fwd_split_on() && N >= 2) {
         const int na = (N + 1) / 2;
         if (par) {
             FOSVOS_HIP_CHECK(hipEventRecord(ev[14], sm));
@@ -184,7 +204,12 @@
                     }
                     FOSVOS_REQUIRE(wsn >= fosvos_conv3x3_workspace_bytes(nf, a.sh[s], a.sw[s], kCin[c], kCout[c]),
                                    FOSVOS_E_WORKSPACE, "vgg_forward: split-K workspace of the second chain");
-                    if (c == kLastOfStage[s] && s < 4) {
+                    if (c == 1 && compact) {
+                        const size_t qpx = (size_t)a.sh[1] * a.sw[1];
+                        FOSVOS_TRY(fosvos_conv3x3_fwd_pool_codes(xh, w->conv_wf[c], w->conv_b[c],
+                                                                 reinterpret_cast<uint16_t *>(base + a.pooled[0]) + (size_t)f0 * qpx * kCout[c],
+                                                                 codes1(f0), nf, H, W, kCin[c], kCout[c], FOSVOS_CONV_RELU, device, st));
+                    } else if (c == kLastOfStage[s] && s < 4) {
                         const size_t qpx = (size_t)a.sh[s + 1] * a.sw[s + 1];
                         FOSVOS_TRY(fosvos_conv3x3_fwd_pool(xh, w->conv_wf[c], w->conv_b[c], yc,
                                                            reinterpret_cast<uint16_t *>(base + a.pooled[s]) + (size_t)f0 * qpx * kCout[c],
@@ -237,7 +262,10 @@
         } else {
             if (c == kFirstOfStage[s])
                 x = reinterpret_cast<uint16_t *>(base + a.pooled[s - 1]);
-            if (c == kLastOfStage[s] && s < 4) {
+            if (c == 1 && compact) {
+                FOSVOS_TRY(fosvos_conv3x3_fwd_pool_codes(x, w->conv_wf[c], w->conv_b[c], reinterpret_cast<uint16_t *>(base + a.pooled[0]),
+                                                         codes1(0), N, H, W, kCin[c], kCout[c], FOSVOS_CONV_RELU, device, stream));
+            } else if (c == kLastOfStage[s] && s < 4) {
                 FOSVOS_TRY(fosvos_conv3x3_fwd_pool(x, w->conv_wf[c], w->conv_b[c], act(c),
                                                    reinterpret_cast<uint16_t *>(base + a.pooled[s]), N, a.sh[s], a.sw[s],
                                                    kCin[c], kCout[c], FOSVOS_CONV_RELU, ws, a.ws_bytes, device, stream));
@@ -278,21 +306,45 @@
 extern "C" int fosvos_vgg_forward_streams(fosvos_ctx *ctx, const fosvos_vgg_weights *w, const float *frame, int N, int H,
                                           int W, void *arena, size_t arena_bytes, float *fused, float *const side_out[4],
                                           void *stream, void *aux_stream) {
+    return fosvos_vgg_forward_streams_flags(ctx, w, frame, N, H, W, arena, arena_bytes, fused, side_out, stream, aux_stream, 0u);
+}
+
+extern "C" int fosvos_vgg_forward_streams_flags(fosvos_ctx *ctx, const fosvos_vgg_weights *w, const float *frame, int N, int H,
+                                                int W, void *arena, size_t arena_bytes, float *fused, float *const side_out[4],
+                                                void *stream, void *aux_stream, unsigned flags) {
     FOSVOS_TRY(ctx_check(ctx, "vgg_forward_streams"));
-    return forward_impl(ctx->vgg_ev, w, frame, N, H, W, arena, arena_bytes, fused, side_out, ctx->device, stream, aux_stream);
-}
+    return forward_impl(ctx->vgg_ev, w, frame, N, H, W, arena, arena_bytes, fused, side_out, ctx->device, stream, aux_stream,
+                        flags);
+}
+
+extern "C" int fosvos_vgg_stage1_compact(unsigned flags, int N, int H, int W) { return stage1_compact(flags, N, H, W) ? 1 : 0; }
 
 extern "C" int fosvos_vgg_forward(const fosvos_vgg_weights *w, const float *frame, int N, int H, int W, void *arena,
                                   size_t arena_bytes, float *fused, float *const side_out[4], int device,
                                   void *stream) {
-    return forward_impl(nullptr, w, frame, N, H, W, arena, arena_bytes, fused, side_out, device, stream, nullptr);
+    return forward_impl(nullptr, w, frame, N, H, W, arena, arena_bytes, fused, side_out, device, stream, nullptr, 0u);
+}
+
+extern "C" int fosvos_vgg_forward_flags(const fosvos_vgg_weights *w, const float *frame, int N, int H, int W, void *arena,
+                                        size_t arena_bytes, float *fused, float *const side_out[4], int device, void *stream,
+                                        unsigned flags) {
+    return forward_impl(nullptr, w, frame, N, H, W, arena, arena_bytes, fused, side_out, device, stream, nullptr, flags);
 }
 
 extern "C" int fosvos_vgg_backward(fosvos_ctx *ctx, const fosvos_vgg_weights *w, const fosvos_vgg_grads *g,
                                    const float *frame, int N, int H, int W, void *arena, size_t arena_bytes,
                                    const float *d_fused, const float *const d_side_out[4], void *stream,
                                    void *aux_stream) {
+    return fosvos_vgg_backward_flags(ctx, w, g, frame, N, H, W, arena, arena_bytes, d_fused, d_side_out, stream, aux_stream, 0u);
+}
+
+extern "C" int fosvos_vgg_backward_flags(fosvos_ctx *ctx, const fosvos_vgg_weights *w, const fosvos_vgg_grads *g,
+                                         const float *frame, int N, int H, int W, void *arena, size_t arena_bytes,
+                                         const float *d_fused, const float *const d_side_out[4], void *stream,
+                                         void *aux_stream, unsigned flags) {
     FOSVOS_TRY(ctx_check(ctx, "vgg_backward"));
+    FOSVOS_REQUIRE((flags & ~FOSVOS_VGG_COMPACT_STAGE1) == 0, FOSVOS_E_ARG, "vgg_backward: unknown flags 0x%x", flags);
+    const bool compact = stage1_compact(flags, N, H, W);
     const int device = ctx->device;
     const Arena a = make_arena(N, H, W);
     FOSVOS_TRY(check_net(w, frame, arena, N, H, W, arena_bytes, a, "vgg_backward"));
@@ -404,7 +456,11 @@
                                       base + a.wsa_conv[c], a.wsa_conv_bytes[c], device, sa,
                                       (offload && s == 1) ? &reduce_m : &reduce, tail && s <= tail_stages));
         }
-        if (s == 1 || (s > 0 && !unpool_fused))
+        if (s == 1 && compact)
+            FOSVOS_TRY(fosvos_maxpool2x2_ceil_bwd_codes(reinterpret_cast<const uint32_t *>(base + a.act[1]),
+                                                        reinterpret_cast<const uint16_t *>(base + a.gpooled[0]), gact(1), N, a.sh[0],
+                                                        a.sw[0], kStageCh[0], device, sm));
+        else if (s == 1 || (s > 0 && !unpool_fused))
             FOSVOS_TRY(fosvos_maxpool2x2_ceil_bwd(act(kLastOfStage[s - 1]), reinterpret_cast<const uint16_t *>(base + a.gpooled[s - 1]),
                                                   gact(kLastOfStage[s - 1]), N, a.sh[s - 1], a.sw[s - 1], kStageCh[s - 1], 1,
                                                   device, sm));
diff --git a/fosvos_amd/fosvos_hip/__init__.py b/fosvos_amd/fosvos_hip/__init__.py
--- a/fosvos_amd/fosvos_hip/__init__.py
+++ b/fosvos_amd/fosvos_hip/__init__.py
@@ -13,6 +13,7 @@
 ABI_VERSION = 33
 CONV_RELU = 1
 CONV_OUT_F32 = 2
+VGG_COMPACT_STAGE1 = 1
 
 
 class FosvosHipError(RuntimeError):
@@ -241,6 +242,17 @@
                                               c_int, c_void_p, ctypes.c_double, c_void_p, c_int, c_void_p]),
     "fosvos_vgg_backward": (c_int, [c_void_p, POINTER(VggWeights), POINTER(VggGrads), c_void_p, c_int, c_int, c_int, c_void_p,
                                     c_size_t, c_void_p, POINTER(c_void_p), c_void_p, c_void_p]),
+    "fosvos_conv3x3_fwd_pool_codes": (c_int, [c_void_p, c_void_p, c_void_p, c_void_p, c_void_p, c_int, c_int, c_int, c_int,
+                                              c_int, c_uint, c_int, c_void_p]),
+    "fosvos_conv3x3_pool_codes_bytes": (c_size_t, [c_int, c_int, c_int, c_int]),
+    "fosvos_maxpool2x2_ceil_bwd_codes": (c_int, [c_void_p, c_void_p, c_void_p, c_int, c_int, c_int, c_int, c_int, c_void_p]),
+    "fosvos_vgg_stage1_compact": (c_int, [c_uint, c_int, c_int, c_int]),
+    "fosvos_vgg_forward_flags": (c_int, [POINTER(VggWeights), c_void_p, c_int, c_int, c_int, c_void_p, c_size_t, c_void_p,
+                                         POINTER(c_void_p), c_int, c_void_p, c_uint]),
+    "fosvos_vgg_forward_streams_flags": (c_int, [c_void_p, POINTER(VggWeights), c_void_p, c_int, c_int, c_int, c_void_p,
+                                                 c_size_t, c_void_p, POINTER(c_void_p), c_void_p, c_void_p, c_uint]),
+    "fosvos_vgg_backward_flags": (c_int, [c_void_p, POINTER(VggWeights), POINTER(VggGrads), c_void_p, c_int, c_int, c_int,
+                                          c_void_p, c_size_t, c_void_p, POINTER(c_void_p), c_void_p, c_void_p, c_uint]),
 }
 
 _lib = None
diff --git a/fosvos_amd/fosvos_hip/engine.py b/fosvos_amd/fosvos_hip/engine.py
--- a/fosvos_amd/fosvos_hip/engine.py
+++ b/fosvos_amd/fosvos_hip/engine.py
@@ -7,7 +7,7 @@
 
 import torch
 
-from . import Context, VggGrads, VggWeights, check, lib, ops, ptr_array4
+from . import VGG_COMPACT_STAGE1, Context, VggGrads, VggWeights, check, lib, ops, ptr_array4
 from .options import EngineOptions, native_loop_from_env
 
 STAGE_CHANNELS = ((64, 64), (128, 128), (256, 256, 256), (512, 512, 512), (512, 512, 512))
@@ -37,14 +37,26 @@
 PARAM_INDEX = {n: i for i, n in enumerate(PARAM_NAMES)}
 
 
+class _PassFlagsSlots:
+    __slots__ = ("_compact_stage1",)
+
+
 @dataclass(slots=True)
-class PassFlags:
+class PassFlags(_PassFlagsSlots):
 
     defer_wgrad_join: bool = False
     forward_one_stream: bool = False
     publish_grad_buckets: bool = False
     overwrite_grads: bool = False
     last_pass_of_cycle: bool = False
+
+    @property
+    def compact_stage1(self) -> bool:
+        return getattr(self, "_compact_stage1", False)
+
+    @compact_stage1.setter
+    def compact_stage1(self, value: bool) -> None:
+        self._compact_stage1 = bool(value)
 
 
 class PackedWeights:
@@ -457,21 +469,23 @@
     opts = packs.options
     aux = (pool.aux_stream(idx) if N >= 2 and opts.fwd_aux and opts.two_streams and not packs.flags.forward_one_stream
            else 0)
+    pass_flags = VGG_COMPACT_STAGE1 if (packs.flags.compact_stage1 and keep) else 0
     if aux:
-        check(lib().fosvos_vgg_forward_streams(pool.ctx(idx), ctypes.byref(w), x.data_ptr(), N, H, W, ap, an, fused.data_ptr(),
-                                               so, torch.cuda.current_stream(idx).cuda_stream, aux), "vgg_forward_streams")
+        check(lib().fosvos_vgg_forward_streams_flags(pool.ctx(idx), ctypes.byref(w), x.data_ptr(), N, H, W, ap, an,
+                                                     fused.data_ptr(), so, torch.cuda.current_stream(idx).cuda_stream, aux,
+                                                     pass_flags), "vgg_forward_streams")
     else:
-        check(lib().fosvos_vgg_forward(ctypes.byref(w), x.data_ptr(), N, H, W, ap, an, fused.data_ptr(), so, idx,
-                                       torch.cuda.current_stream(idx).cuda_stream), "vgg_forward")
+        check(lib().fosvos_vgg_forward_flags(ctypes.byref(w), x.data_ptr(), N, H, W, ap, an, fused.data_ptr(), so, idx,
+                                             torch.cuda.current_stream(idx).cuda_stream, pass_flags), "vgg_forward")
     ops._pe(t0, "vgg_forward", 2.0 * 129.114e9 * N * H * W / (480 * 854), 0.0)
     if not keep:
         pool.give(N, H, W, arena)
         arena = None
-    return (outs if outs is not None else [None] * 4) + [fused], (arena, x, w, keep_alive, (N, H, W))
+    return (outs if outs is not None else [None] * 4) + [fused], (arena, x, w, keep_alive, (N, H, W), pass_flags)
 
 
 def native_backward(P, packs, saved, d_outs, inplace: bool) -> Dict[str, torch.Tensor]:
-    arena, x, w, keep_alive, (N, H, W) = saved
+    arena, x, w, keep_alive, (N, H, W), pass_flags = saved
     dev = x.device
     d_fused = d_outs[4]
     d_so, with_so = _side_grads(d_outs)
@@ -521,9 +535,9 @@
         dso = ptr_array4([t.data_ptr() for t in d_so])
     ap, an = _aligned_ptr(arena)
     t0 = ops._pb()
-    check(lib().fosvos_vgg_backward(packs.arenas.ctx(idx), ctypes.byref(w), ctypes.byref(g), x.data_ptr(), N, H, W, ap, an,
-                                    d_fused.data_ptr() if d_fused is not None else None, dso,
-                                    torch.cuda.current_stream(idx).cuda_stream, aux or None),
+    check(lib().fosvos_vgg_backward_flags(packs.arenas.ctx(idx), ctypes.byref(w), ctypes.byref(g), x.data_ptr(), N, H, W, ap, an,
+                                          d_fused.data_ptr() if d_fused is not None else None, dso,
+                                          torch.cuda.current_stream(idx).cuda_stream, aux or None, pass_flags),
           "vgg_backward")
     ops._pe(t0, "vgg_backward", 2.0 * (2 * 129.114e9 - 0.708e9) * N * H * W / (480 * 854), 0.0)
     if with_so:
diff --git a/fosvos_amd/fosvos_hip/ops.py b/fosvos_amd/fosvos_hip/ops.py
--- a/fosvos_amd/fosvos_hip/ops.py
+++ b/fosvos_amd/fosvos_hip/ops.py
@@ -291,6 +291,41 @@
     return y, yp
 
 
+def conv3x3_pool_codes_shape(n: int, h: int, w: int, c: int) -> Tuple[int, int, int, int]:
+    return (n, (h + 1) // 2, (w + 1) // 2, c // 8)
+
+
+def conv3x3_fwd_pool_codes(x: torch.Tensor, w_packed: torch.Tensor, bias: Optional[torch.Tensor], ci: int, co: int,
+                           out: Optional[Tuple[torch.Tensor, torch.Tensor]] = None) -> Tuple[torch.Tensor, torch.Tensor]:
+    _need(x, _BF16, "conv3x3_fwd_pool_codes x"); _need(w_packed, _BF16, "conv3x3_fwd_pool_codes packed weight")
+    n, h, wd, cx = x.shape
+    if cx != _ru(ci, 32):
+        raise ValueError(f"conv3x3_fwd_pool_codes: x has {cx} channels, expected {_ru(ci, 32)}")
+    L = lib()
+    if w_packed.numel() != L.fosvos_packed_weight_elems(co, ci):
+        raise ValueError("conv3x3_fwd_pool_codes: packed weight size does not match (Co, Ci)")
+    if bias is not None:
+        _need(bias, _F32, "conv3x3_fwd_pool_codes bias")
+        if bias.numel() != co:
+            raise ValueError("conv3x3_fwd_pool_codes: bias size")
+    if out is None:
+        yp = torch.empty((n, (h + 1) // 2, (wd + 1) // 2, co), dtype=_BF16, device=x.device)
+        codes = torch.empty(conv3x3_pool_codes_shape(n, h, wd, co), dtype=torch.int32, device=x.device)
+    else:
+        yp, codes = out
+        _need(yp, _BF16, "conv3x3_fwd_pool_codes pooled output")
+        if not (codes.is_cuda and codes.is_contiguous() and codes.dtype == torch.int32):
+            raise ValueError("conv3x3_fwd_pool_codes: codes must be a contiguous int32 tensor on the GPU")
+        if yp.numel() != n * ((h + 1) // 2) * ((wd + 1) // 2) * co or codes.numel() * 4 != L.fosvos_conv3x3_pool_codes_bytes(n, h, wd, co):
+            raise ValueError("conv3x3_fwd_pool_codes: output sizes")
+    dev, st = _ctx(x)
+    t0 = _pb()
+    check(L.fosvos_conv3x3_fwd_pool_codes(x.data_ptr(), w_packed.data_ptr(), _p(bias), yp.data_ptr(), codes.data_ptr(), n, h,
+                                          wd, ci, co, CONV_RELU, dev, st), "conv3x3_fwd_pool_codes")
+    _pe(t0, "conv3x3_fwd", 2.0 * n * h * wd * 9 * ci * co, n * h * wd * 2 * cx + 2 * 9 * ci * co + yp.numel() * 2 + codes.numel() * 4)
+    return yp, codes
+
+
 def conv3x3_dgrad(dy: torch.Tensor, w_dgrad_packed: torch.Tensor, ci: int, co: int,
                   relu_src: Optional[torch.Tensor] = None, addend: Optional[torch.Tensor] = None,
                   out: Optional[torch.Tensor] = None, relu_bits: Optional[torch.Tensor] = None) -> torch.Tensor:
@@ -417,6 +452,31 @@
                                            dev, st), "maxpool2x2_ceil_bwd")
     _pe(t0, "maxpool_bwd", 0.0, 2 * (2 * x.numel() + dy.numel()))
     return dx
+
+
+def maxpool_bwd_codes(codes: torch.Tensor, dy: torch.Tensor, h: int, w: int, out: Optional[torch.Tensor] = None) -> torch.Tensor:
+    _need(dy, _BF16, "maxpool_bwd_codes dy")
+    n, oh, ow, c = dy.shape
+    if (oh, ow) != ((h + 1) // 2, (w + 1) // 2) or c % 8:
+        raise ValueError("maxpool_bwd_codes: dy shape mismatch")
+    if not (codes.is_cuda and codes.is_contiguous() and codes.dtype == torch.int32) or codes.numel() != n * oh * ow * (c // 8):
+        raise ValueError("maxpool_bwd_codes: codes must be a contiguous int32 [N, ceil(h/2), ceil(w/2), C/8] tensor on the GPU")
+    dx = torch.empty((n, h, w, c), dtype=_BF16, device=dy.device) if out is None else out
+    if out is not None:
+        _need(out, _BF16, "maxpool_bwd_codes out")
+        if out.numel() != n * h * w * c:
+            raise ValueError("maxpool_bwd_codes: out size")
+    dev, st = _ctx(dy)
+    t0 = _pb()
+    check(lib().fosvos_maxpool2x2_ceil_bwd_codes(codes.data_ptr(), dy.data_ptr(), dx.data_ptr(), n, h, w, c, dev, st),
+          "maxpool2x2_ceil_bwd_codes")
+    _pe(t0, "maxpool_bwd", 0.0, 2 * (dx.numel() + dy.numel()) + 4 * codes.numel())
+    return dx
+
+
+def vgg_stage1_compact(n: int, h: int, w: int, flag: bool = True) -> bool:
+    from . import VGG_COMPACT_STAGE1
+    return bool(lib().fosvos_vgg_stage1_compact(VGG_COMPACT_STAGE1 if flag else 0, n, h, w))
 
 
 def head_fwd(side: Sequence[torch.Tensor], filt: Sequence[torch.Tensor], filt1: Optional[Sequence[torch.Tensor]],
diff --git a/fosvos_amd/networks/osvos_vgg.py b/fosvos_amd/networks/osvos_vgg.py
--- a/fosvos_amd/networks/osvos_vgg.py
+++ b/fosvos_amd/networks/osvos_vgg.py
@@ -198,3 +198,4 @@
 
 for _field in dataclasses.fields(engine.PassFlags):
     setattr(OSVOS_VGG, _field.name, _pass_flag(_field.name))
+OSVOS_VGG.compact_stage1 = _pass_flag('compact_stage1')
diff --git a/fosvos_amd/train_offline.py b/fosvos_amd/train_offline.py
--- a/fosvos_amd/train_offline.py
+++ b/fosvos_amd/train_offline.py
@@ -99,7 +99,7 @@
 def _train(net_provider: NetworkProvider, data_loader_train, data_loader_test, optimizer: optim.SGD, summary_writer,
            start_epoch: int, n_epochs: int, avg_grad_every_n: int, snapshot_every_n: int,
            is_testing_while_training: bool, test_every_n: int, *, options: Optional[LoopOptions] = None,
-           microbatch_group: int = 1) -> dict:
+           microbatch_group: int = 1, compact_stage1: bool = True) -> dict:
     if options is None:
         options = LoopOptions.from_env()
     microbatch_group = int(microbatch_group)
@@ -189,6 +189,7 @@
         net.join_gradients()
     flags.defer_wgrad_join = options.defer_join
     try:
+        flags.compact_stage1 = bool(compact_stage1)
         for epoch in range(start_epoch, n_epochs):
             start_time = timeit.default_timer()
             sampler = getattr(data_loader_train, 'sampler', None)
@@ -243,6 +244,7 @@
     finally:
         net.join_gradients()
         flags.defer_wgrad_join = False
+        flags.compact_stage1 = False
         if microbatch_group > 1 and reserved_frames is not None:
             net.reserve_arena_frames = reserved_frames
     if torch.cuda.is_available():
diff --git a/fosvos_amd/train_online.py b/fosvos_amd/train_online.py
--- a/fosvos_amd/train_online.py
+++ b/fosvos_amd/train_online.py
@@ -287,7 +287,7 @@
 
 def _train(net_provider: NetworkProvider, dataloader, optimizer: optim.SGD, summary_writer, seq_name: str,
            start_epoch: int, n_epochs: int, avg_grad_every_n: int, snapshot_every_n: int, *,
-           options: Optional[LoopOptions] = None) -> dict:
+           options: Optional[LoopOptions] = None, compact_stage1: bool = True) -> dict:
     if options is None:
         options = LoopOptions.from_env()
     log.info('Start of Online Training, sequence: ' + seq_name)
@@ -468,6 +468,7 @@
         net.join_gradients()
     flags.defer_wgrad_join = options.defer_join
     try:
+        flags.compact_stage1 = bool(compact_stage1)
         window = []
         for epoch in range(start_epoch, n_epochs):
             n_mb = len(dataloader)
@@ -489,6 +490,7 @@
             if grads_stale:
                 flat.zero()
         flags.forward_one_stream = False
+        flags.compact_stage1 = False
         net.compute_side_outputs = True
     time_enqueued = timeit.default_timer() - time_all_start
     if torch.cuda.is_available():
diff --git a/include/fosvos_hip.h b/include/fosvos_hip.h
--- a/include/fosvos_hip.h
+++ b/include/fosvos_hip.h
@@ -87,6 +87,10 @@
 int fosvos_conv3x3_fwd_pool(const uint16_t *x, const uint16_t *w_packed, const float *bias, uint16_t *y,
                             uint16_t *y_pool, int N, int H, int W, int Ci, int Co, unsigned flags, void *workspace,
                             size_t workspace_bytes, int device, void *stream);
+int fosvos_conv3x3_fwd_pool_codes(const uint16_t *x, const uint16_t *w_packed, const float *bias, uint16_t *y_pool,
+                                  uint32_t *codes, int N, int H, int W, int Ci, int Co, unsigned flags, int device,
+                                  void *stream);
+size_t fosvos_conv3x3_pool_codes_bytes(int N, int H, int W, int C);
 size_t fosvos_conv3x3_workspace_bytes(int N, int H, int W, int in_ch, int out_ch);
 typedef struct fosvos_conv3x3_plan_info {
     int tile_h, tile_w, tile_co;
@@ -117,6 +121,8 @@
 int fosvos_maxpool2x2_ceil_fwd(const uint16_t *x, uint16_t *y, int N, int H, int W, int C, int device, void *stream);
 int fosvos_maxpool2x2_ceil_bwd(const uint16_t *x, const uint16_t *dy, uint16_t *dx, int N, int H, int W, int C,
                                int relu_mask, int device, void *stream);
+int fosvos_maxpool2x2_ceil_bwd_codes(const uint32_t *codes, const uint16_t *dy, uint16_t *dx, int N, int H, int W, int C,
+                                     int device, void *stream);
 
 int fosvos_head_fwd(const float *const side[4], const int hs[4], const int ws[4], const float *const filt[4],
                     const float *const filt1[4], const float *dsn_w , const float *dsn_b ,
@@ -337,6 +343,17 @@
 int fosvos_vgg_backward(fosvos_ctx *ctx, const fosvos_vgg_weights *w, const fosvos_vgg_grads *g, const float *frame, int N,
                         int H, int W, void *arena, size_t arena_bytes, const float *d_fused,
                         const float *const d_side_out[4], void *stream, void *aux_stream);
+#define FOSVOS_VGG_COMPACT_STAGE1 1u
+int fosvos_vgg_stage1_compact(unsigned flags, int N, int H, int W);
+int fosvos_vgg_forward_flags(const fosvos_vgg_weights *w, const float *frame, int N, int H, int W, void *arena,
+                             size_t arena_bytes, float *fused, float *const side_out[4], int device, void *stream,
+                             unsigned flags);
+int fosvos_vgg_forward_streams_flags(fosvos_ctx *ctx, const fosvos_vgg_weights *w, const float *frame, int N, int H, int W,
+                                     void *arena, size_t arena_bytes, float *fused, float *const side_out[4], void *stream,
+                                     void *aux_stream, unsigned flags);
+int fosvos_vgg_backward_flags(fosvos_ctx *ctx, const fosvos_vgg_weights *w, const fosvos_vgg_grads *g, const float *frame,
+                              int N, int H, int W, void *arena, size_t arena_bytes, const float *d_fused,
+                              const float *const d_side_out[4], void *stream, void *aux_stream, unsigned flags);
 int fosvos_vgg_grad_bucket_wait(fosvos_ctx *ctx, int bucket, void *stream);
 
 #ifdef __cplusplus
```

After: 1272 frames/s, median of 6. +1.8%, better.
